# whxhcj/multimodal-S2UT

Measured on AMD Instinct MI355X. Metric: audio-frames/sec/node, mm_s2ut_transformer fp16, max-tokens 40000, 1/2/4/8 GPUs, higher is better.
Workload: dtype fp16; 1 GPU; mm_s2ut_transformer base (ViT-768 image feats, multimodal_attention+gate); model=mm_s2ut_transformer, parallelism=dp1, front_end=GPU fbank+CMVN in step

## Files before the change

### include/mms2ut.h

```cpp
#ifndef MMS2UT_H
#define MMS2UT_H

#include <hip/hip_runtime.h>
#include <stdint.h>

#ifdef __cplusplus
extern "C" {
#endif

typedef _Float16 mms2ut_half;

const char* mms2ut_last_error(void);
int mms2ut_stream_create(int priority, hipStream_t* out);
int mms2ut_stream_destroy(hipStream_t stream);
int mms2ut_version(void);

enum {
  MMS_EPI_F16 = 0,
  MMS_EPI_RELU_DROP = 1,
  MMS_EPI_DROP_RESID = 2,
  MMS_EPI_F32 = 3,
  MMS_EPI_GATE = 4,
  MMS_EPI_RELU_DROP_BWD = 5,
  MMS_EPI_F16_ACC = 6,
// ... 29 lines not shown
} mms2ut_gemm_args;

int mms2ut_gemm_f16(const mms2ut_gemm_args* args, hipStream_t stream);
int mms2ut_gemm_set_tall(int mode);

int mms2ut_gemm_set_skinny(int mode);
int mms2ut_gemm_skinny_debug(int scatter, int* xcc_out);
int mms2ut_gemm_set_epilogue(int staged);

typedef struct mms2ut_wgrad {
  const mms2ut_half* dy;
  int64_t lddy;
  const mms2ut_half* x;
  int64_t ldx;
  mms2ut_half* dW;
  mms2ut_half* db;
  int N, K;
} mms2ut_wgrad;
int mms2ut_wgrad_group(const mms2ut_wgrad* w, int n, int64_t rows, int max_blocks, hipStream_t stream);

int mms2ut_profile_begin(int max_launches);
int mms2ut_profile_end(float* total_ms, int* launches, double* flops);
int mms2ut_profile_bytes(double* bytes);
int mms2ut_profile_launches(float* ms, double* flops, int* cls, int n);
int mms2ut_profile_shapes(int* mnk, int n);
int mms2ut_profile_stamps(unsigned long long* stamps, long cap_blocks);
int mms2ut_profile_blocks(long* first_last, int n);
int mms2ut_wallclock_khz(int* khz);

int mms2ut_splitk_reduce(const float* slabs, int nsplit, int64_t slab, int rows, int cols,
                         void* out, int64_t ldo, int mode, float alpha, hipStream_t stream);
int mms2ut_splitk_reduce_bias(const float* slabs, int nsplit, int64_t slab, int rows, int cols,
                              mms2ut_half* out, int64_t ldo, const float* rs_slabs,
                              mms2ut_half* rs_out, hipStream_t stream);

typedef struct mms2ut_transpose_desc {
  int64_t src, dst;
  int32_t rows, cols, tile0, pad;
} mms2ut_transpose_desc;
int mms2ut_transpose_batch(const mms2ut_half* src, mms2ut_half* dst, const mms2ut_transpose_desc* descs,
                           int n, int total_tiles, hipStream_t stream);

int mms2ut_stream_wait(hipStream_t waiter, hipStream_t signaler);
int mms2ut_event_create(hipEvent_t* out);
int mms2ut_event_record(hipEvent_t event, hipStream_t stream);
int mms2ut_event_wait(hipStream_t stream, hipEvent_t event);
int mms2ut_event_destroy(hipEvent_t event);
int mms2ut_bind_step_seed(const uint64_t* delta);
int mms2ut_step_seed_advance(uint64_t* delta, uint64_t inc, hipStream_t stream);

int mms2ut_layernorm_fwd(const mms2ut_half* x, const mms2ut_half* gamma, const mms2ut_half* beta,
                         mms2ut_half* y, float* mean, float* rstd, int64_t rows, int D, float eps,
                         hipStream_t stream);
int mms2ut_layernorm_bwd(const mms2ut_half* dy, const mms2ut_half* x, const mms2ut_half* gamma,
                         const float* mean, const float* rstd, const mms2ut_half* dres,
                         mms2ut_half* dx, float* part, int64_t rows, int D, mms2ut_half* dxd,
                         float p, uint64_t seed, uint64_t offset, hipStream_t stream);
int mms2ut_layernorm_bwd_parts(int64_t rows);
int mms2ut_layernorm_bwd_nparts(int64_t rows, int D);
int mms2ut_layernorm_fwd_ex(const mms2ut_half* x, const mms2ut_half* gamma, const mms2ut_half* beta,
                            mms2ut_half* y, float* mean, float* rstd, int64_t rows, int D, float eps,
                            int64_t grp, int64_t grp_out, float p, uint64_t seed, uint64_t offset,
                            hipStream_t stream);
int mms2ut_layernorm_bwd_ex(const mms2ut_half* dy, const mms2ut_half* x, const mms2ut_half* gamma,
                            const float* mean, const float* rstd, const mms2ut_half* dres,
                            mms2ut_half* dx, float* part, int64_t rows, int D, mms2ut_half* dxd,
                            float p, uint64_t seed, uint64_t offset, int64_t dy_grp, int64_t dy_grp_out,
                            float dy_p, uint64_t dy_seed, uint64_t dy_offset, hipStream_t stream);
int mms2ut_colsum_parts(const float* part, int nparts, int ncol, mms2ut_half* out, int accumulate,
                        hipStream_t stream);
int mms2ut_colsum_f16(const mms2ut_half* x, int64_t rows, int cols, int64_t ld, float* part,
                      int nparts, hipStream_t stream);
int mms2ut_colsum_nparts(int64_t rows);

int mms2ut_attn_softmax_fwd(const mms2ut_half* S, mms2ut_half* P, mms2ut_half* Pd, int Z, int H,
                            int Tq, int Tk, int64_t ldS, const int32_t* key_len,
                            const uint8_t* key_mask, int64_t ld_mask, int causal,
                            int extra_key, float p, uint64_t seed, uint64_t offset,
                            hipStream_t stream);
int mms2ut_attn_softmax_bwd(const mms2ut_half* P, const mms2ut_half* dPd, mms2ut_half* dS, int Z,
                            int H, int Tq, int Tk, int64_t ldS, const int32_t* key_len, int causal,
                            int extra_key, float p, uint64_t seed, uint64_t offset,
                            hipStream_t stream);

typedef struct mms2ut_attn_args {
  const mms2ut_half* q;
  const mms2ut_half* k;
  const mms2ut_half* v;
  mms2ut_half* o;
  int64_t ldq, ldk, ldv, ldo;
  int64_t sqb, skb, svb, sob;
  int B, H, Tq, Tk, hd;
  const int32_t* key_len;
  int causal;
  float scale;
  float p;
  uint64_t seed, offset;
  float* lse;
} mms2ut_attn_args;

int mms2ut_mha_varlen_fwd(const mms2ut_attn_args* args, hipStream_t stream);
int mms2ut_mha_varlen_bwd(const mms2ut_attn_args* args, const mms2ut_half* dout, int64_t lddo,
                          int64_t sdob, float* Dd, mms2ut_half* dq, int64_t lddq, int64_t sdqb,
                          mms2ut_half* dk, int64_t lddk, int64_t sdkb, mms2ut_half* dv,
                          int64_t lddv, int64_t sdvb, hipStream_t stream);

int mms2ut_dropout_fwd(const mms2ut_half* x, mms2ut_half* y, int64_t n, float p, uint64_t seed,
                       uint64_t offset, hipStream_t stream);
int mms2ut_dropout_mask(uint8_t* keep, int64_t n, float p, uint64_t seed, uint64_t offset,
                        hipStream_t stream);
int mms2ut_encoder_embed_fwd(const mms2ut_half* h, const mms2ut_half* pos_table, const int32_t* len,
                             mms2ut_half* x, int B, int T, int D, float scale, float p,
                             uint64_t seed, uint64_t offset, hipStream_t stream);
int mms2ut_scale_dropout_bwd(const mms2ut_half* dx, mms2ut_half* dh, int64_t n, float scale,
                             float p, uint64_t seed, uint64_t offset, hipStream_t stream);
int mms2ut_token_embed_fwd(const int64_t* tok, const mms2ut_half* E, const mms2ut_half* pos_table,
                           mms2ut_half* x, int B, int T, int D, int pad_idx, float scale, float p,
                           uint64_t seed, uint64_t offset, hipStream_t stream);
int mms2ut_token_embed_bwd(const int64_t* tok, const mms2ut_half* dx, float* dE32, int B, int T,
                           int D, int V, int pad_idx, float scale, float p, uint64_t seed,
                           uint64_t offset, hipStream_t stream);
int mms2ut_add_f32_to_f16(const mms2ut_half* a, const float* b, mms2ut_half* out, int64_t n,
                          hipStream_t stream);
int mms2ut_glu_fwd(const mms2ut_half* x, mms2ut_half* y, int64_t rows, int C, hipStream_t stream);
int mms2ut_glu_bwd(const mms2ut_half* x, const mms2ut_half* dy, mms2ut_half* dx, int64_t rows,
                   int C, hipStream_t stream);
int mms2ut_im2col(const mms2ut_half* x, mms2ut_half* col, int B, int Tin, int Tout, int C, int k,
                  int stride, int pad, hipStream_t stream);
int mms2ut_im2col_ld(const mms2ut_half* x, mms2ut_half* col, int B, int Tin, int Tout, int C, int k,
                     int stride, int pad, int ldcol, hipStream_t stream);
int mms2ut_col2im(const mms2ut_half* dcol, mms2ut_half* dx, int B, int Tin, int Tout, int C, int k,
                  int stride, int pad, hipStream_t stream);
int mms2ut_gate_bwd(const mms2ut_half* dres, const mms2ut_half* merge, const mms2ut_half* g,
                    mms2ut_half* dpre, mms2ut_half* dmerge, int64_t rows, int D,
                    hipStream_t stream);
int mms2ut_copy2d(const mms2ut_half* src, int64_t lds, mms2ut_half* dst, int64_t ldd, int64_t rows,
                  int cols, hipStream_t stream);
int mms2ut_copy2d_pad(const mms2ut_half* src, int64_t lds, mms2ut_half* dst, int64_t ldd, int64_t rows,
                      int cols, int zcols, hipStream_t stream);
int mms2ut_add_f16(const mms2ut_half* a, const mms2ut_half* b, mms2ut_half* out, int64_t n,
                   hipStream_t stream);

#define MMS_LS_XENT_PARTS 512
int mms2ut_ls_xent_fwd(const mms2ut_half* logits, int64_t ld, const int64_t* target, int64_t rows,
                       int V, float eps, int pad_idx, float* lse, float* part, float* loss_out,
                       hipStream_t stream);
int mms2ut_ls_xent_fwd_log(const mms2ut_half* logits, int64_t ld, const int64_t* target, int64_t rows,
                           int V, float eps, int pad_idx, float* lse, float* part, float* acc, float* call_out,
                           hipStream_t stream);
int mms2ut_ls_xent_bwd(const mms2ut_half* logits, int64_t ld, const int64_t* target, int64_t rows,
                       int V, float eps, int pad_idx, const float* lse, const float* grad,
                       mms2ut_half* dlogits, hipStream_t stream);

enum {
  MMS_OST_MULT = 0, MMS_OST_GNORM = 1, MMS_OST_OVERFLOW = 2, MMS_OST_STEP = 3,
  MMS_OST_STEP_SIZE = 4, MMS_OST_LOSS_SCALE = 5, MMS_OST_ITER = 6, MMS_OST_LAST_OVERFLOW = 7,
  MMS_OST_LAST_RESCALE = 8, MMS_OST_CLIP_COEF = 9, MMS_OST_FATAL = 10, MMS_OST_LR = 11,
  MMS_OST_INCONSISTENT = 12, MMS_OST_SIZE = 16
};
int mms2ut_grad_sqnorm(const mms2ut_half* grad, int64_t n, float* part, int nparts,
                       hipStream_t stream);
int mms2ut_grad_norm_finalize(const float* part, int nparts, float* ost, const float* sample_size,
                              hipStream_t stream);
int mms2ut_optim_prepare(float* ost, float lr, float warmup_init_lr, float warmup_updates, float beta1,
                         float beta2, float clip_norm, float scale_window, float min_loss_scale,
                         hipStream_t stream);
// ... 46 lines not shown
int mms2ut_specaugment_f16(mms2ut_half* x, const int32_t* frame_off, int B, int Tmax, int nbins,
                           const int32_t* masks, int n_freq, int n_time, int use_const,
                           float mask_value, hipStream_t stream);
#define MMS_NOISE_SPLIT    8
#define MMS_NOISE_MAX_MIX  4
#define MMS_NOISE_WS_DOUBLES(B) ((int64_t)3 * (B) * MMS_NOISE_SPLIT)
int mms2ut_noise_mix_f32(float* wave, const int64_t* wave_off, int B,
                         const int16_t* bank, const int64_t* bank_off, int n_clips,
                         const int32_t* params, int n_mix, double* ws, hipStream_t stream);

enum { MMS_LAYER_ENC = 0, MMS_LAYER_DEC = 1 };
enum {
  MMS_SLOT_M1 = 0, MMS_SLOT_R1, MMS_SLOT_H1, MMS_SLOT_QKV, MMS_SLOT_LSE_SA, MMS_SLOT_O, MMS_SLOT_XA,
  MMS_SLOT_M2, MMS_SLOT_R2, MMS_SLOT_H2, MMS_SLOT_Q, MMS_SLOT_LSE_CA, MMS_SLOT_CO, MMS_SLOT_XB,
  MMS_SLOT_M3, MMS_SLOT_R3, MMS_SLOT_H3, MMS_SLOT_F1, MMS_SLOT_OUT, MMS_LAYER_NSLOT
};

typedef struct mms2ut_layer {
  int kind;
  int B, T, Tk, d, H, F;
  float eps;
  const int32_t* self_len;
  const int32_t* cross_len;
  const mms2ut_half *ln1_g, *ln1_b, *w_qkv, *b_qkv, *w_o, *b_o;
  const mms2ut_half *ln2_g, *ln2_b, *w_cq, *b_cq, *w_co, *b_co;
  const mms2ut_half* kv;
  int64_t ld_kv;
  const mms2ut_half *ln3_g, *ln3_b, *w_fc1, *b_fc1, *w_fc2, *b_fc2;
  const mms2ut_half *wt_qkv, *wt_o, *wt_cq, *wt_co, *wt_fc1, *wt_fc2;
  mms2ut_half *g_ln1, *g_w_qkv, *g_b_qkv, *g_w_o, *g_b_o;
  mms2ut_half *g_ln2, *g_w_cq, *g_b_cq, *g_w_co, *g_b_co;
  mms2ut_half *g_ln3, *g_w_fc1, *g_b_fc1, *g_w_fc2, *g_b_fc2;
  float p_drop, p_attn, p_act;
  uint64_t seed;
  uint64_t off_sa_attn, off_sa_res, off_ca_attn, off_ca_res, off_act, off_ffn_res;
  const mms2ut_half* x;
  void* saved;
} mms2ut_layer;

typedef struct mms2ut_layer_grad {
  const mms2ut_half* dy;
  const mms2ut_half* dy_drop;
  float emit_p;
  uint64_t emit_seed, emit_offset;
  mms2ut_half* dkv;
  int64_t ld_dkv;
  void* scratch;
  float* main_ws;
  int64_t main_ws_floats;
  float* side_ws;
  int64_t side_ws_floats;
  int side_blocks;
} mms2ut_layer_grad;

int mms2ut_layer_arena(const mms2ut_layer* layer, int64_t* offsets, int64_t* bytes);
int mms2ut_layer_scratch(const mms2ut_layer* layer, float emit_p, int64_t* dx_offsets, int64_t* bytes);
int mms2ut_layer_ws(const mms2ut_layer* layer, int64_t* main_floats, int64_t* side_floats);
int mms2ut_layer_fwd(const mms2ut_layer* layer, float* main_ws, int64_t main_ws_floats, hipStream_t stream);
int mms2ut_layer_bwd(const mms2ut_layer* layer, const mms2ut_layer_grad* grad, hipStream_t main,
                     hipStream_t side);
int mms2ut_wgrad_flush(hipStream_t main);

#define MMS_CONV_MAX 4
typedef struct mms2ut_conv1d_glu {
  int B, T, C, nlayers;
  int k[MMS_CONV_MAX];
  int cout[MMS_CONV_MAX];
  const mms2ut_half* w[MMS_CONV_MAX];
  const mms2ut_half* b[MMS_CONV_MAX];
  const mms2ut_half* wt[MMS_CONV_MAX];
  mms2ut_half* g_w[MMS_CONV_MAX];
  mms2ut_half* g_b[MMS_CONV_MAX];
  const mms2ut_half* x;
  void* saved;
} mms2ut_conv1d_glu;
int mms2ut_conv1d_glu_arena(const mms2ut_conv1d_glu* c, int64_t* out_offset, int64_t* bytes);
int mms2ut_conv1d_glu_scratch(const mms2ut_conv1d_glu* c, int64_t* dx_offset, int64_t* bytes);
int mms2ut_conv1d_glu_ws(const mms2ut_conv1d_glu* c, int64_t* main_floats, int64_t* side_floats);
int mms2ut_conv1d_glu_fwd(const mms2ut_conv1d_glu* c, float* main_ws, int64_t main_ws_floats, hipStream_t stream);
int mms2ut_conv1d_glu_bwd(const mms2ut_conv1d_glu* c, const mms2ut_half* dy, void* scratch, float* main_ws,
                          int64_t main_ws_floats, float* side_ws, int64_t side_ws_floats, int side_blocks,
                          hipStream_t main, hipStream_t side);

typedef struct mms2ut_gated_fusion {
  int B, Te, Ti, Di, d;
  int extra;
  int gate;
  int image_pre_norm;
  float eps;
  float p_img, p_txt, p_attn;
  uint64_t seed, off_img, off_txt, off_attn;
  const uint8_t* key_mask;
  int64_t ld_mask;
  const mms2ut_half *ln_g, *ln_b, *wq, *bq, *wkv, *bkv, *bias_kv, *wo, *bo, *wg, *bg;
  mms2ut_half *g_ln, *g_wq, *g_bq, *g_wkv, *g_bkv, *g_bias_kv, *g_wo, *g_bo, *g_wg, *g_bg;
  const mms2ut_half *wt_q, *wt_kv, *wt_o, *wt_g;
  const mms2ut_half* text;
  const mms2ut_half* img;
  void* saved;
} mms2ut_gated_fusion;
int mms2ut_gated_fusion_arena(const mms2ut_gated_fusion* f, int64_t* out_offset, int64_t* bytes);
int mms2ut_gated_fusion_scratch(const mms2ut_gated_fusion* f, int want_dimg, int64_t* offsets, int64_t* bytes);
int mms2ut_gated_fusion_ws(const mms2ut_gated_fusion* f, int64_t* main_floats, int64_t* side_floats);
int mms2ut_gated_fusion_fwd(const mms2ut_gated_fusion* f, float* main_ws, int64_t main_ws_floats, hipStream_t stream);
int mms2ut_gated_fusion_bwd(const mms2ut_gated_fusion* f, const mms2ut_half* dres, int want_dimg, void* scratch,
                            float* main_ws, int64_t main_ws_floats, float* side_ws, int64_t side_ws_floats,
                            int side_blocks, hipStream_t main, hipStream_t side);

enum { MMS_OP_LAYER = 0, MMS_OP_CONV1D_GLU = 1, MMS_OP_GATED_FUSION = 2 };
int mms2ut_workspace_size(int op, const void* desc, int64_t* sizes);

#ifdef __cplusplus
}
#endif
#endif
```

### multimodal-s2ut_amd/_lib.py

```python
import ctypes as C
import os
import struct

HERE = os.path.dirname(os.path.abspath(__file__))
LIB_PATH = os.environ.get("MMS2UT_LIB") or os.path.join(HERE, "lib", "libmms2ut_hip.so")

vp, i32, i64, u64, f32 = C.c_void_p, C.c_int, C.c_int64, C.c_uint64, C.c_float

EPI_F16, EPI_RELU_DROP, EPI_DROP_RESID, EPI_F32, EPI_GATE, EPI_RELU_DROP_BWD, EPI_F16_ACC, EPI_GELU_DROP, \
    EPI_GELU_DROP_BWD = range(9)


class GemmArgs(C.Structure):
    _fields_ = [
        ("A", vp), ("B", vp), ("C", vp),
        ("M", i32), ("N", i32), ("K", i32),
        ("a_kcontig", i32), ("b_kcontig", i32),
        ("lda", i64), ("ldb", i64), ("ldc", i64),
        ("batch", i32), ("bdiv", i32),
        ("sA1", i64), ("sA2", i64), ("sB1", i64), ("sB2", i64), ("sC1", i64), ("sC2", i64),
        ("splitk", i32),
        ("sCsplit", i64),
        ("epi", i32),
        ("alpha", f32),
# ... 58 lines not shown


CONV_MAX = 4


class ConvArgs(C.Structure):
    _fields_ = [("B", i32), ("T", i32), ("C", i32), ("nlayers", i32), ("k", i32 * CONV_MAX), ("cout", i32 * CONV_MAX)] + \
        [(n, vp * CONV_MAX) for n in ("w", "b", "wt", "g_w", "g_b")] + [("x", vp), ("saved", vp)]


class FusionArgs(C.Structure):
    _fields_ = [(n, i32) for n in ("B", "Te", "Ti", "Di", "d", "extra", "gate", "image_pre_norm")] + \
        [(n, f32) for n in ("eps", "p_img", "p_txt", "p_attn")] + [(n, u64) for n in ("seed", "off_img", "off_txt", "off_attn")] + \
        [("key_mask", vp), ("ld_mask", i64)] + \
        [(n, vp) for n in ("ln_g", "ln_b", "wq", "bq", "wkv", "bkv", "bias_kv", "wo", "bo", "wg", "bg",
                           "g_ln", "g_wq", "g_bq", "g_wkv", "g_bkv", "g_bias_kv", "g_wo", "g_bo", "g_wg", "g_bg",
                           "wt_q", "wt_kv", "wt_o", "wt_g", "text", "img", "saved")]


OP_LAYER, OP_CONV1D_GLU, OP_GATED_FUSION = range(3)


class WgradArgs(C.Structure):
    _fields_ = [("dy", vp), ("lddy", i64), ("x", vp), ("ldx", i64), ("dW", vp), ("db", vp), ("N", i32), ("K", i32)]


class LayerGradArgs(C.Structure):
    _fields_ = [("dy", vp), ("dy_drop", vp), ("emit_p", f32), ("emit_seed", u64), ("emit_offset", u64),
                ("dkv", vp), ("ld_dkv", i64), ("scratch", vp), ("main_ws", vp), ("main_ws_floats", i64),
                ("side_ws", vp), ("side_ws_floats", i64), ("side_blocks", i32)]


LAYER_GRAD_ARGS = _packer(LayerGradArgs)


SIGNATURES = {
    "mms2ut_last_error": (C.c_char_p, []),
    "mms2ut_version": (i32, []),
    "mms2ut_stream_create": (i32, [i32, vp]),
    "mms2ut_stream_destroy": (i32, [vp]),
    "mms2ut_event_create": (i32, [vp]),
    "mms2ut_event_record": (i32, [vp, vp]),
    "mms2ut_event_wait": (i32, [vp, vp]),
    "mms2ut_event_destroy": (i32, [vp]),
    "mms2ut_gemm_f16": (i32, [vp, vp]),
    "mms2ut_gemm_set_tall": (i32, [i32]),
    "mms2ut_gemm_set_skinny": (i32, [i32]),
    "mms2ut_gemm_skinny_debug": (i32, [i32, vp]),
    "mms2ut_gemm_set_epilogue": (i32, [i32]),
    "mms2ut_wgrad_group": (i32, [vp, i32, i64, i32, vp]),
    "mms2ut_wgrad_flush": (i32, [vp]),
    "mms2ut_profile_begin": (i32, [i32]),
    "mms2ut_profile_end": (i32, [C.POINTER(C.c_float), C.POINTER(C.c_int), C.POINTER(C.c_double)]),
    "mms2ut_profile_bytes": (i32, [C.POINTER(C.c_double)]),
    "mms2ut_profile_launches": (i32, [C.c_void_p, C.c_void_p, C.c_void_p, i32]),
    "mms2ut_profile_shapes": (i32, [C.c_void_p, i32]),
    "mms2ut_profile_stamps": (i32, [vp, C.c_long]),
    "mms2ut_profile_blocks": (i32, [C.c_void_p, i32]),
    "mms2ut_wallclock_khz": (i32, [C.POINTER(C.c_int)]),
    "mms2ut_grad_norm_check": (i32, [vp, i32, i32, vp, i32, vp]),
    "mms2ut_ctc_workspace_floats": (i32, [i32, i32, i32, C.POINTER(C.c_int64)]),
    "mms2ut_ctc_loss_fwd": (i32, [vp, i64, i32, i32, i32, vp, i64, i32, vp, vp, i32, i32, vp, vp, vp]),
    "mms2ut_ctc_loss_bwd": (i32, [vp, i64, i32, i32, i32, vp, i64, i32, vp, vp, i32, vp, vp, vp, i64, vp]),
    "mms2ut_scale_f16": (i32, [vp, i64, f32, vp]),
    "mms2ut_accum_f16_f32": (i32, [vp, vp, i64, vp]),
    "mms2ut_set_f32": (i32, [vp, i32, vp, vp]),
    "mms2ut_splitk_reduce": (i32, [vp, i32, i64, i32, i32, vp, i64, i32, f32, vp]),
    "mms2ut_splitk_reduce_bias": (i32, [vp, i32, i64, i32, i32, vp, i64, vp, vp, vp]),
    "mms2ut_transpose_batch": (i32, [vp, vp, vp, i32, i32, vp]),
    "mms2ut_layernorm_fwd": (i32, [vp, vp, vp, vp, vp, vp, i64, i32, f32, vp]),
    "mms2ut_layernorm_bwd": (i32, [vp, vp, vp, vp, vp, vp, vp, vp, i64, i32, vp, f32, u64, u64, vp]),
    "mms2ut_layernorm_bwd_parts": (i32, [i64]),
    "mms2ut_layernorm_bwd_nparts": (i32, [i64, i32]),
    "mms2ut_layernorm_fwd_ex": (i32, [vp, vp, vp, vp, vp, vp, i64, i32, f32, i64, i64, f32, u64, u64, vp]),
    "mms2ut_layernorm_bwd_ex": (i32, [vp, vp, vp, vp, vp, vp, vp, vp, i64, i32, vp, f32, u64, u64, i64, i64,
                                      f32, u64, u64, vp]),
    "mms2ut_colsum_parts": (i32, [vp, i32, i32, vp, i32, vp]),
    "mms2ut_colsum_f16": (i32, [vp, i64, i32, i64, vp, i32, vp]),
    "mms2ut_colsum_nparts": (i32, [i64]),
    "mms2ut_attn_softmax_fwd": (i32, [vp, vp, vp, i32, i32, i32, i32, i64, vp, vp, i64, i32, i32,
                                      f32, u64, u64, vp]),
    "mms2ut_attn_softmax_bwd": (i32, [vp, vp, vp, i32, i32, i32, i32, i64, vp, i32, i32, f32, u64,
                                      u64, vp]),
    "mms2ut_mha_varlen_fwd": (i32, [vp, vp]),
    "mms2ut_mha_varlen_bwd": (i32, [vp, vp, i64, i64, vp, vp, i64, i64, vp, i64, i64,
                                    vp, i64, i64, vp]),
    "mms2ut_dropout_fwd": (i32, [vp, vp, i64, f32, u64, u64, vp]),
    "mms2ut_dropout_mask": (i32, [vp, i64, f32, u64, u64, vp]),
    "mms2ut_encoder_embed_fwd": (i32, [vp, vp, vp, vp, i32, i32, i32, f32, f32, u64, u64, vp]),
    "mms2ut_scale_dropout_bwd": (i32, [vp, vp, i64, f32, f32, u64, u64, vp]),
    "mms2ut_token_embed_fwd": (i32, [vp, vp, vp, vp, i32, i32, i32, i32, f32, f32, u64, u64, vp]),
    "mms2ut_token_embed_bwd": (i32, [vp, vp, vp, i32, i32, i32, i32, i32, f32, f32, u64, u64, vp]),
    "mms2ut_add_f32_to_f16": (i32, [vp, vp, vp, i64, vp]),
    "mms2ut_add_f16": (i32, [vp, vp, vp, i64, vp]),
    "mms2ut_glu_fwd": (i32, [vp, vp, i64, i32, vp]),
    "mms2ut_glu_bwd": (i32, [vp, vp, vp, i64, i32, vp]),
    "mms2ut_im2col": (i32, [vp, vp, i32, i32, i32, i32, i32, i32, i32, vp]),
    "mms2ut_im2col_ld": (i32, [vp, vp, i32, i32, i32, i32, i32, i32, i32, i32, vp]),
    "mms2ut_col2im": (i32, [vp, vp, i32, i32, i32, i32, i32, i32, i32, vp]),
    "mms2ut_gate_bwd": (i32, [vp, vp, vp, vp, vp, i64, i32, vp]),
    "mms2ut_copy2d_pad": (i32, [vp, i64, vp, i64, i64, i32, i32, vp]),
    "mms2ut_copy2d": (i32, [vp, i64, vp, i64, i64, i32, vp]),
    "mms2ut_ls_xent_fwd": (i32, [vp, i64, vp, i64, i32, f32, i32, vp, vp, vp, vp]),
    "mms2ut_ls_xent_fwd_log": (i32, [vp, i64, vp, i64, i32, f32, i32, vp, vp, vp, vp, vp]),
    "mms2ut_ls_xent_bwd": (i32, [vp, i64, vp, i64, i32, f32, i32, vp, vp, vp, vp]),
    "mms2ut_grad_sqnorm": (i32, [vp, i64, vp, i32, vp]),
    "mms2ut_grad_norm_finalize": (i32, [vp, i32, vp, vp, vp]),
    "mms2ut_stream_wait": (i32, [vp, vp]),
    "mms2ut_bind_step_seed": (i32, [vp]),
    "mms2ut_step_seed_advance": (i32, [vp, u64, vp]),
    "mms2ut_optim_prepare": (i32, [vp, f32, f32, f32, f32, f32, f32, f32, f32, vp]),
    "mms2ut_adam_fp16_master": (i32, [vp, vp, vp, vp, vp, i64, vp, f32, f32, f32, f32, vp]),
    "mms2ut_fbank_frames": (i32, [vp, i32, vp, vp]),
    "mms2ut_fbank_f32": (i32, [vp, vp, vp, i32, i32, vp, vp, i32, vp, vp]),
    "mms2ut_fbank_cmvn_collate": (i32, [vp, vp, i32, i32, i32, i32, vp, vp, vp]),
    "mms2ut_specaugment_f16": (i32, [vp, vp, i32, i32, i32, vp, i32, i32, i32, f32, vp]),
    "mms2ut_noise_mix_f32": (i32, [vp, vp, i32, vp, vp, i32, vp, i32, vp, vp]),
    "mms2ut_layer_arena": (i32, [vp, vp, vp]),
    "mms2ut_layer_scratch": (i32, [vp, f32, vp, vp]),
    "mms2ut_layer_ws": (i32, [vp, vp, vp]),
    "mms2ut_layer_fwd": (i32, [vp, vp, i64, vp]),
    "mms2ut_layer_bwd": (i32, [vp, vp, vp, vp]),
    "mms2ut_gated_fusion_arena": (i32, [vp, vp, vp]),
    "mms2ut_gated_fusion_scratch": (i32, [vp, i32, vp, vp]),
    "mms2ut_gated_fusion_ws": (i32, [vp, vp, vp]),
    "mms2ut_gated_fusion_fwd": (i32, [vp, vp, i64, vp]),
    "mms2ut_gated_fusion_bwd": (i32, [vp, vp, i32, vp, vp, i64, vp, i64, i32, vp, vp]),
    "mms2ut_workspace_size": (i32, [i32, vp, vp]),
    "mms2ut_conv1d_glu_arena": (i32, [vp, vp, vp]),
    "mms2ut_conv1d_glu_scratch": (i32, [vp, vp, vp]),
    "mms2ut_conv1d_glu_ws": (i32, [vp, vp, vp]),
    "mms2ut_conv1d_glu_fwd": (i32, [vp, vp, i64, vp]),
    "mms2ut_conv1d_glu_bwd": (i32, [vp, vp, vp, vp, i64, vp, i64, i32, vp, vp]),
    "mms2ut_log_softmax_step": (i32, [vp, i64, i64, i32, i32, i32, i32, vp, vp]),
    "mms2ut_kv_cache_gather": (i32, [vp, vp, vp, i32, i32, i32, i32, i32, i32, vp]),
    "mms2ut_decode_self_attn": (i32, [vp, i64, vp, vp, i32, i32, i32, i32, vp, vp, i64, i64, vp, i64, f32, vp]),
    "mms2ut_decode_embed": (i32, [vp, vp, vp, vp, i32, vp, i32, i32, f32, vp]),
    "mms2ut_splitk_epilogue_f16": (i32, [vp, i32, i64, i32, i32, vp, vp, i64, i32, vp, i64, vp]),
    "mms2ut_beam_topk": (i32, [vp, vp, i64, i32, i32, i32, i32, i32, vp, vp, vp, vp, vp]),
    "mms2ut_splitk_epilogue_ln_f16": (i32, [vp, i32, i64, i32, i32, vp, vp, i64, vp, i64, vp, vp, f32, vp, i64,
                                            vp]),
}

_lib = None


class HipError(RuntimeError):
    pass


def load():
    global _lib
    if _lib is not None:
        return _lib
    if not os.path.exists(LIB_PATH):
        raise HipError(f"libmms2ut_hip.so not found at {LIB_PATH}; run "
                       f"`python multimodal-s2ut_amd/build.py` (hipcc, gfx950)")
    lib = C.CDLL(LIB_PATH)
    for name, (res, args) in SIGNATURES.items():
        fn = getattr(lib, name)
        fn.restype = res
        fn.argtypes = args
    _lib = lib
    return lib


def call(name, *args):
    rc = getattr(_lib or load(), name)(*args)
    if rc != 0:
        raise HipError(f"{name} failed ({rc}): {_lib.mms2ut_last_error().decode()}")
    return rc
```

### multimodal-s2ut_amd/csrc/layers.hip

```cpp
#include <math.h>
#include <stdlib.h>

#include <algorithm>

#include "common.h"
#include "../../include/mms2ut.h"

namespace {

constexpr int64_t kAlign = 256;

int64_t al(int64_t b) { return (b + kAlign - 1) / kAlign * kAlign; }

struct Dims {
  bool dec;
  int64_t R, Rk, d, F, BHT, BHTk;
};

Dims dims_of(const mms2ut_layer* L) {
  Dims D;
  D.dec = L->kind == MMS_LAYER_DEC;
  D.R = (int64_t)L->B * L->T;
  D.Rk = (int64_t)L->B * L->Tk;
  D.d = L->d;
// ... 560 lines not shown
    const int k = c->k[i], N = c->cout[i];
    mms2ut_half* col = at<mms2ut_half>(A, off, i * CA_N + CA_COL);
    mms2ut_half* y = at<mms2ut_half>(A, off, i * CA_N + CA_Y);
    mms2ut_half* g = at<mms2ut_half>(A, off, i * CA_N + CA_G);
    if ((rc = mms2ut_im2col_ld(x, col, c->B, (int)D.Tin[i], (int)D.Tout[i], (int)D.C[i], k, 2, k / 2, (int)D.kp[i], s)))
      return rc;
    const mms2ut_half* W = c->w[i];
    if (D.kp[i] != D.ck[i]) {
      mms2ut_half* Wp = at<mms2ut_half>(A, off, i * CA_N + CA_WP);
      if ((rc = mms2ut_copy2d_pad(W, D.ck[i], Wp, D.kp[i], N, (int)D.ck[i], (int)(D.kp[i] - D.ck[i]), s))) return rc;
      W = Wp;
    }
    if ((rc = linear(cx, col, W, c->b[i], y, D.rows[i], N, D.kp[i]))) return rc;
    if ((rc = mms2ut_glu_fwd(y, g, D.rows[i], N / 2, s))) return rc;
    x = g;
  }
  return 0;
}

extern "C" int mms2ut_conv1d_glu_bwd(const mms2ut_conv1d_glu* c, const mms2ut_half* dy, void* scratch,
                                     float* main_ws, int64_t main_ws_floats, float* side_ws,
                                     int64_t side_ws_floats, int side_blocks, hipStream_t main, hipStream_t side) {
  if (int rc = conv_check(c)) return rc;
  MMS_REQUIRE(dy && scratch && c->saved, "conv1d_glu_bwd: null gradient / scratch / arena");
  if (!side) side = main;
  const ConvDims D = conv_dims(c);
  int64_t sz[MMS_CONV_MAX * CA_N], off[MMS_CONV_MAX * CA_N];
  conv_arena_sizes(c, D, sz);
  layout(sz, MMS_CONV_MAX * CA_N, off);
  int64_t ssz[MMS_CONV_MAX * CS_N + 1], so[MMS_CONV_MAX * CS_N + 1];
  conv_scratch_sizes(c, D, ssz);
  layout(ssz, MMS_CONV_MAX * CS_N + 1, so);
  void* A = c->saved;
  void* S = scratch;
  const Ctx cx{main, side, main_ws, main_ws_floats, side_ws, side_ws_floats, at<float>(S, so, MMS_CONV_MAX * CS_N),
               nullptr, nullptr, false};
  const mms2ut_half* dg = dy;
  int rc;
  for (int i = D.n - 1; i >= 0; --i) {
    const int k = c->k[i], N = c->cout[i];
    const mms2ut_half* col = at<mms2ut_half>(A, off, i * CA_N + CA_COL);
    mms2ut_half* dyi = at<mms2ut_half>(S, so, i * CS_N + CS_DY);
    if ((rc = mms2ut_glu_bwd(at<mms2ut_half>(A, off, i * CA_N + CA_Y), dg, dyi, D.rows[i], N / 2, main))) return rc;
    if (c->g_w[i]) {
      if (conv_group_ok(c, D, i)) {
        if ((rc = fork(cx))) return rc;
        mms2ut_wgrad w{dyi, N, col, D.kp[i], c->g_w[i], c->g_b[i], N, (int)D.ck[i]};
        if ((rc = mms2ut_wgrad_group(&w, 1, D.rows[i], side == main ? 0 : side_blocks, side))) return rc;
      } else if ((rc = wgrad(cx, dyi, N, col, D.kp[i], c->g_w[i], c->g_b[i], D.rows[i], N, D.ck[i]))) {
        return rc;
      }
    }
    if (i == 0) break;
    mms2ut_half* dcol = at<mms2ut_half>(S, so, i * CS_N + CS_DCOL);
    mms2ut_half* dx = at<mms2ut_half>(S, so, i * CS_N + CS_DX);
    if ((rc = dgrad(cx, dyi, N, c->w[i], c->wt[i], dcol, D.rows[i], N, D.ck[i]))) return rc;
    if ((rc = mms2ut_col2im(dcol, dx, c->B, (int)D.Tin[i], (int)D.Tout[i], (int)D.C[i], k, 2, k / 2, main))) return rc;
    dg = dx;
  }
  return 0;
}

namespace {

bool wgrad_group_ok(const mms2ut_half* dy, int64_t lddy, const mms2ut_half* x, int64_t ldx, const mms2ut_half* dW,
                    int64_t M, int64_t N, int64_t K) {
  auto al16 = [](const void* p) { return ((uintptr_t)p & 15) == 0; };
  return ((N + 127) / 128) * ((K + 127) / 128) >= 256 && N % 8 == 0 && K % 8 == 0 && lddy % 8 == 0 && ldx % 8 == 0 &&
         al16(dy) && al16(x) && al16(dW) && M * std::max(lddy, ldx) * 2 < (1LL << 31);
}

int wgrad_auto(const Ctx& c, const mms2ut_half* dy, int64_t lddy, const mms2ut_half* x, int64_t ldx, mms2ut_half* dW,
               mms2ut_half* db, int64_t M, int64_t N, int64_t K, int side_blocks) {
  if (wgrad_group_ok(dy, lddy, x, ldx, dW, M, N, K)) {
    int rc = fork(c);
    if (rc) return rc;
    mms2ut_wgrad w{dy, lddy, x, ldx, dW, db, (int)N, (int)K};
    return mms2ut_wgrad_group(&w, 1, M, c.side == c.main ? 0 : side_blocks, c.side);
  }
  return wgrad(c, dy, lddy, x, ldx, dW, db, M, N, K);
}

struct FusDims {
  int64_t B, Te, Ti, Tk, Di, d, Rt, Ri, Rk, ldS;
  bool extra, gate, pre, ln_fused;
};

FusDims fus_dims(const mms2ut_gated_fusion* f) {
  FusDims D;
  D.B = f->B; D.Te = f->Te; D.Ti = f->Ti; D.Di = f->Di; D.d = f->d;
  D.extra = f->extra != 0; D.gate = f->gate != 0; D.pre = f->image_pre_norm != 0;
  D.Tk = D.Ti + (D.extra ? 1 : 0);
  D.Rt = D.B * D.Te; D.Ri = D.B * D.Ti; D.Rk = D.B * D.Tk;
  D.ldS = (D.Tk + 7) / 8 * 8;
  D.ln_fused = D.pre && D.Di % 256 == 0 && D.Di <= 1024;
  return D;
}

enum { FA_IM = 0, FA_IR, FA_IMGN, FA_IMGD, FA_TEXTD, FA_Q, FA_KV, FA_S, FA_P, FA_PD, FA_O, FA_MERGE, FA_G, FA_OUT, FA_N };
void fus_arena_sizes(const mms2ut_gated_fusion* f, const FusDims& D, int64_t* sz) {
  for (int i = 0; i < FA_N; ++i) sz[i] = 0;
  const int64_t h = 2;
  if (D.pre) sz[FA_IM] = sz[FA_IR] = D.Ri * 4;
  if (!D.ln_fused && (D.pre || f->p_img > 0.f)) sz[FA_IMGN] = D.Ri * D.Di * h;
  if (D.ln_fused || D.extra) sz[FA_IMGD] = D.Rk * D.Di * h;
  if (f->p_txt > 0.f) sz[FA_TEXTD] = D.Rt * D.d * h;
  sz[FA_Q] = D.Rt * D.d * h;
  sz[FA_KV] = D.Rk * 2 * D.d * h;
  sz[FA_S] = sz[FA_P] = D.Rt * D.ldS * h;
  if (f->p_attn > 0.f) sz[FA_PD] = sz[FA_P];
  sz[FA_O] = D.Rt * D.d * h;
  if (D.gate) { sz[FA_MERGE] = D.Rt * 2 * D.d * h; sz[FA_G] = D.Rt * D.d * h; }
  sz[FA_OUT] = D.Rt * D.d * h;
}

enum { FS_DPRE = 0, FS_DMERGE, FS_DO, FS_DQ, FS_DKV, FS_DPD, FS_DIMGD, FS_DIMG, FS_DIMGIN, FS_DTEXT, FS_LNP, FS_KVP,
       FS_BPART, FS_N };
void fus_scratch_sizes(const mms2ut_gated_fusion* f, const FusDims& D, int want_dimg, int64_t* sz) {
  for (int i = 0; i < FS_N; ++i) sz[i] = 0;
  const int64_t h = 2;
  if (D.gate) { sz[FS_DPRE] = D.Rt * D.d * h; sz[FS_DMERGE] = D.Rt * 2 * D.d * h; }
  sz[FS_DO] = sz[FS_DQ] = D.Rt * D.d * h;
  sz[FS_DKV] = D.Rk * 2 * D.d * h;
  sz[FS_DPD] = D.Rt * D.ldS * h;
  if (D.pre || want_dimg) {
    sz[FS_DIMGD] = D.Rk * D.Di * h;
    sz[FS_DIMG] = D.Ri * D.Di * h;
    sz[FS_DIMGIN] = D.Ri * D.Di * h;
    if (D.pre) sz[FS_LNP] = (int64_t)mms2ut_layernorm_bwd_nparts(D.Ri, (int)D.Di) * 2 * D.Di * 4;
  }
  sz[FS_DTEXT] = D.Rt * D.d * h;
  if (D.extra) sz[FS_KVP] = (int64_t)mms2ut_colsum_nparts(D.B) * 2 * D.d * 4;
  sz[FS_BPART] = (int64_t)mms2ut_colsum_nparts(std::max(D.Rt, D.Rk)) * 2 * D.d * 4;
}

int fus_check(const mms2ut_gated_fusion* f) {
  MMS_REQUIRE(f && f->B >= 1 && f->Te >= 1 && f->Ti >= 1, "gated_fusion: B, Te, Ti must be >= 1");
  MMS_REQUIRE(f->d % 8 == 0 && f->Di % 8 == 0 && f->d > 0 && f->Di > 0, "gated_fusion: d=%d Di=%d (multiples of 8)", f->d, f->Di);
  MMS_REQUIRE(f->wq && f->bq && f->wkv && f->bkv && f->wo && f->bo, "gated_fusion: projection weights / biases required");
  MMS_REQUIRE(!f->extra || f->bias_kv, "gated_fusion: multimodal attention needs bias_kv");
  MMS_REQUIRE(!f->gate || (f->wg && f->bg), "gated_fusion: the gate needs its weight and bias");
  MMS_REQUIRE(!f->image_pre_norm || (f->ln_g && f->ln_b), "gated_fusion: image_pre_norm needs the LayerNorm");
  return 0;
}

mms2ut_gemm_args batched(const mms2ut_half* A, const mms2ut_half* B_, void* C, int M, int N, int K, int a_kc, int b_kc,
                         int64_t lda, int64_t ldb, int64_t ldc, int batch, int64_t sA, int64_t sB, int64_t sC,
                         float alpha) {
  mms2ut_gemm_args a = gemm_args();
  a.A = A; a.B = B_; a.C = C;
  a.M = M; a.N = N; a.K = K;
  a.a_kcontig = a_kc; a.b_kcontig = b_kc;
  a.lda = lda; a.ldb = ldb; a.ldc = ldc;
  a.batch = batch; a.bdiv = 1;
  a.sA1 = sA; a.sB1 = sB; a.sC1 = sC;
  a.sA2 = a.sB2 = a.sC2 = 0;
  a.alpha = alpha;
  return a;
}

int zero_rows(mms2ut_half* p, int64_t pitch_elems, int64_t width_elems, int64_t rows, hipStream_t s) {
  return mms2ut_copy2d_pad(nullptr, 0, p, pitch_elems, rows, 0, (int)width_elems, s);
}

}

extern "C" int mms2ut_gated_fusion_arena(const mms2ut_gated_fusion* f, int64_t* out_offset, int64_t* bytes) {
  if (int rc = fus_check(f)) return rc;
  MMS_REQUIRE(bytes, "gated_fusion_arena: null");
  const FusDims D = fus_dims(f);
  int64_t sz[FA_N], off[FA_N];
  fus_arena_sizes(f, D, sz);
  *bytes = layout(sz, FA_N, off);
  if (out_offset) *out_offset = off[FA_OUT];
  return 0;
}

extern "C" int mms2ut_gated_fusion_scratch(const mms2ut_gated_fusion* f, int want_dimg, int64_t* offsets, int64_t* bytes) {
  if (int rc = fus_check(f)) return rc;
  MMS_REQUIRE(bytes, "gated_fusion_scratch: null");
  const FusDims D = fus_dims(f);
  int64_t sz[FS_N], off[FS_N];
  fus_scratch_sizes(f, D, want_dimg, sz);
  *bytes = layout(sz, FS_N, off);
  if (offsets) {
    offsets[0] = off[FS_DTEXT];
    offsets[1] = want_dimg ? (D.pre ? off[FS_DIMGIN] : (D.extra ? off[FS_DIMG] : off[FS_DIMGD])) : -1;
  }
  return 0;
}

extern "C" int mms2ut_gated_fusion_ws(const mms2ut_gated_fusion* f, int64_t* main_floats, int64_t* side_floats) {
  if (int rc = fus_check(f)) return rc;
  MMS_REQUIRE(main_floats && side_floats, "gated_fusion_ws: null");
  const FusDims D = fus_dims(f);
  int64_t mw = 0, sw = 0;
  auto fw = [&](int64_t M, int64_t N, int64_t K) {
    const int s = fixup_splits(M, N, K);
    if (s > 1) mw = std::max(mw, (int64_t)s * M * N);
  };
  auto ww = [&](int64_t M, int64_t N, int64_t K) {
    const int s = wgrad_splits(((N + 127) / 128) * ((K + 127) / 128), M);
    sw = std::max(sw, (int64_t)s * N * K + (int64_t)s * N);
  };
  const int64_t d = D.d;
  fw(D.Rt, d, d); fw(D.Rk, 2 * d, D.Di); fw(D.Rt, d, d); fw(D.Rt, d, 2 * d);
  fw(D.Rt, 2 * d, d); fw(D.Rt, d, d); fw(D.Rk, D.Di, 2 * d); fw(D.Rt, d, d);
  ww(D.Rt, d, 2 * d); ww(D.Rt, d, d); ww(D.Rk, 2 * d, D.Di); ww(D.Rt, d, d);
  *main_floats = mw;
  *side_floats = sw;
  return 0;
}

extern "C" int mms2ut_gated_fusion_fwd(const mms2ut_gated_fusion* f, float* main_ws, int64_t main_ws_floats,
                                       hipStream_t s) {
  if (int rc = fus_check(f)) return rc;
  MMS_REQUIRE(f->text && f->img && f->saved, "gated_fusion_fwd: null text / image / arena");
  const FusDims D = fus_dims(f);
  int64_t sz[FA_N], off[FA_N];
  fus_arena_sizes(f, D, sz);
  layout(sz, FA_N, off);
  void* A = f->saved;
  auto H_ = [&](int slot) { return at<mms2ut_half>(A, off, slot); };
  const Ctx c{s, s, main_ws, main_ws_floats, nullptr, 0, nullptr};
  const int64_t d = D.d, Di = D.Di;
  int rc;
  const mms2ut_half* imgd;
  if (D.ln_fused) {
    if (D.extra && (rc = zero_rows(H_(FA_IMGD) + D.Ti * Di, D.Tk * Di, Di, D.B, s))) return rc;
    if ((rc = mms2ut_layernorm_fwd_ex(f->img, f->ln_g, f->ln_b, H_(FA_IMGD), at<float>(A, off, FA_IM),
                                      at<float>(A, off, FA_IR), D.Ri, (int)Di, f->eps, D.extra ? D.Ti : 0,
                                      D.extra ? D.Tk : 0, f->p_img, f->seed, f->off_img, s))) return rc;
    imgd = H_(FA_IMGD);
  } else {
    const mms2ut_half* imgn = f->img;
    if (D.pre) {
      if ((rc = mms2ut_layernorm_fwd(f->img, f->ln_g, f->ln_b, H_(FA_IMGN), at<float>(A, off, FA_IM),
                                     at<float>(A, off, FA_IR), D.Ri, (int)Di, f->eps, s))) return rc;
      imgn = H_(FA_IMGN);
    }
    if (f->p_img > 0.f) {
      if ((rc = mms2ut_dropout_fwd(imgn, H_(FA_IMGN), D.Ri * Di, f->p_img, f->seed, f->off_img, s))) return rc;
      imgn = H_(FA_IMGN);
    }
    if (D.extra) {
      if ((rc = mms2ut_copy2d_pad(imgn, D.Ti * Di, H_(FA_IMGD), D.Tk * Di, D.B, (int)(D.Ti * Di),
                                  (int)((D.Tk - D.Ti) * Di), s)))
        return rc;
      imgd = H_(FA_IMGD);
    } else {
      imgd = imgn;
    }
  }
  const mms2ut_half* textd = f->text;
  if (f->p_txt > 0.f) {
    if ((rc = mms2ut_dropout_fwd(f->text, H_(FA_TEXTD), D.Rt * d, f->p_txt, f->seed, f->off_txt, s))) return rc;
    textd = H_(FA_TEXTD);
  }
  mms2ut_half *q = H_(FA_Q), *kv = H_(FA_KV), *O = H_(FA_O);
  if ((rc = linear(c, textd, f->wq, f->bq, q, D.Rt, d, d))) return rc;
  if ((rc = linear(c, imgd, f->wkv, f->bkv, kv, D.Rk, 2 * d, Di))) return rc;
  if (D.extra && (rc = mms2ut_copy2d(f->bias_kv, 0, kv + D.Ti * 2 * d, D.Tk * 2 * d, D.B, (int)(2 * d), s))) return rc;
  const float scale = (float)pow((double)d, -0.5);
  mms2ut_half *S = H_(FA_S), *P = H_(FA_P), *Pd = f->p_attn > 0.f ? H_(FA_PD) : P;
  {
    mms2ut_gemm_args a = batched(q, kv, S, (int)D.Te, (int)D.Tk, (int)d, 1, 1, d, 2 * d, D.ldS, (int)D.B, D.Te * d,
                                 D.Tk * 2 * d, D.Te * D.ldS, scale);
    if ((rc = mms2ut_gemm_f16(&a, s))) return rc;
  }
  if ((rc = mms2ut_attn_softmax_fwd(S, P, Pd, (int)D.B, 1, (int)D.Te, (int)D.Tk, D.ldS, nullptr, f->key_mask,
                                    f->key_mask ? f->ld_mask : 0, 0, D.extra ? 1 : 0, f->p_attn,
                                    f->p_attn > 0.f ? f->seed : 0, f->p_attn > 0.f ? f->off_attn : 0, s))) return rc;
  {
    mms2ut_gemm_args a = batched(Pd, kv + d, O, (int)D.Te, (int)d, (int)D.Tk, 1, 0, D.ldS, 2 * d, d, (int)D.B,
                                 D.Te * D.ldS, D.Tk * 2 * d, D.Te * d, 1.f);
    if ((rc = mms2ut_gemm_f16(&a, s))) return rc;
  }
  mms2ut_half* out = H_(FA_OUT);
  if (D.gate) {
    mms2ut_half* merge = H_(FA_MERGE);
    if ((rc = gemm_nt(c, O, d, f->wo, d, 1, merge, 2 * d, D.Rt, d, d, MMS_EPI_F16, f->bo, nullptr, 0, 0.f, 0, 0, d)))
      return rc;
    if ((rc = mms2ut_copy2d(textd, d, merge + d, 2 * d, D.Rt, (int)d, s))) return rc;
    mms2ut_gemm_args a = gemm_args();
    a.A = merge; a.B = f->wg; a.C = out;
    a.M = (int)D.Rt; a.N = (int)d; a.K = (int)(2 * d);
    a.a_kcontig = 1; a.b_kcontig = 1;
    a.lda = 2 * d; a.ldb = 2 * d; a.ldc = d;
    a.epi = MMS_EPI_GATE; a.bias = f->bg; a.aux = merge; a.ldaux = 2 * d; a.out2 = H_(FA_G); a.ldo2 = d;
    a.ld_rng = d;
    const int sp = fixup_splits(D.Rt, d, 2 * d);
    if (sp > 1) {
      MMS_REQUIRE(main_ws && main_ws_floats >= (int64_t)sp * D.Rt * d, "gated_fusion_fwd: main workspace too small");
      a.splitk = sp; a.splitk_ws = main_ws; a.splitk_ws_floats = main_ws_floats;
    }
    return mms2ut_gemm_f16(&a, s);
  }
  return linear(c, O, f->wo, f->bo, out, D.Rt, d, d, MMS_EPI_DROP_RESID, textd);
}

extern "C" int mms2ut_gated_fusion_bwd(const mms2ut_gated_fusion* f, const mms2ut_half* dres, int want_dimg,
                                       void* scratch, float* main_ws, int64_t main_ws_floats, float* side_ws,
                                       int64_t side_ws_floats, int side_blocks, hipStream_t main, hipStream_t side) {
  if (int rc = fus_check(f)) return rc;
  MMS_REQUIRE(dres && scratch && f->saved, "gated_fusion_bwd: null gradient / scratch / arena");
  if (!side) side = main;
  const FusDims D = fus_dims(f);
  int64_t sz[FA_N], off[FA_N], ssz[FS_N], so[FS_N];
  fus_arena_sizes(f, D, sz);
  layout(sz, FA_N, off);
  fus_scratch_sizes(f, D, want_dimg, ssz);
  layout(ssz, FS_N, so);
  void* A = f->saved;
  void* S = scratch;
  auto H_ = [&](int slot) { return at<mms2ut_half>(A, off, slot); };
  auto SH = [&](int slot) { return at<mms2ut_half>(S, so, slot); };
  auto SF = [&](int slot) { return at<float>(S, so, slot); };
  const Ctx c{main, side, main_ws, main_ws_floats, side_ws, side_ws_floats, SF(FS_BPART), nullptr, nullptr, false};
  const int64_t d = D.d, Di = D.Di;
  const mms2ut_half* textd = f->p_txt > 0.f ? H_(FA_TEXTD) : f->text;
  const mms2ut_half* imgd = (D.ln_fused || D.extra) ? H_(FA_IMGD) : (!D.ln_fused && (D.pre || f->p_img > 0.f) ? H_(FA_IMGN) : f->img);
  int rc;
  const mms2ut_half *dOp = dres, *dtext = dres;
  int64_t lddop = d, lddtext = d;
  if (D.gate) {
    mms2ut_half *dpre = SH(FS_DPRE), *dmerge = SH(FS_DMERGE);
    if ((rc = mms2ut_gate_bwd(dres, H_(FA_MERGE), H_(FA_G), dpre, dmerge, D.Rt, (int)d, main))) return rc;
    if ((rc = wgrad_auto(c, dpre, d, H_(FA_MERGE), 2 * d, f->g_wg, f->g_bg, D.Rt, d, 2 * d, side_blocks))) return rc;
    if ((rc = dgrad(c, dpre, d, f->wg, f->wt_g, dmerge, D.Rt, d, 2 * d, MMS_EPI_F16_ACC))) return rc;
    dOp = dmerge; lddop = 2 * d;
    dtext = dmerge + d; lddtext = 2 * d;
  }
  if ((rc = wgrad_auto(c, dOp, lddop, H_(FA_O), d, f->g_wo, f->g_bo, D.Rt, d, d, side_blocks))) return rc;
  mms2ut_half* dO = SH(FS_DO);
  if ((rc = dgrad(c, dOp, lddop, f->wo, f->wt_o, dO, D.Rt, d, d))) return rc;
  const float scale = (float)pow((double)d, -0.5);
  const mms2ut_half *q = H_(FA_Q), *kv = H_(FA_KV), *P = H_(FA_P), *Pd = f->p_attn > 0.f ? H_(FA_PD) : P;
  mms2ut_half *dq = SH(FS_DQ), *dkv = SH(FS_DKV), *dPd = SH(FS_DPD);
  const int B = (int)D.B, Te = (int)D.Te, Tk = (int)D.Tk;
  const int64_t sS = D.Te * D.ldS;
  {
    mms2ut_gemm_args a = batched(dO, kv + d, dPd, Te, Tk, (int)d, 1, 1, d, 2 * d, D.ldS, B, D.Te * d, D.Tk * 2 * d, sS, 1.f);
    if ((rc = mms2ut_gemm_f16(&a, main))) return rc;
    a = batched(Pd, dO, dkv + d, Tk, (int)d, Te, 0, 0, D.ldS, d, 2 * d, B, sS, D.Te * d, D.Tk * 2 * d, 1.f);
    if ((rc = mms2ut_gemm_f16(&a, main))) return rc;
  }
  if ((rc = mms2ut_attn_softmax_bwd(P, dPd, dPd, B, 1, Te, Tk, D.ldS, nullptr, 0, 0, f->p_attn,
                                    f->p_attn > 0.f ? f->seed : 0, f->p_attn > 0.f ? f->off_attn : 0, main))) return rc;
  {
    mms2ut_gemm_args a = batched(dPd, kv, dq, Te, (int)d, Tk, 1, 0, D.ldS, 2 * d, d, B, sS, D.Tk * 2 * d, D.Te * d, scale);
    if ((rc = mms2ut_gemm_f16(&a, main))) return rc;
    a = batched(dPd, q, dkv, Tk, (int)d, Te, 0, 0, D.ldS, d, 2 * d, B, sS, D.Te * d, D.Tk * 2 * d, scale);
    if ((rc = mms2ut_gemm_f16(&a, main))) return rc;
  }
  if (D.extra) {
    mms2ut_half* rows = dkv + D.Ti * 2 * d;
    const int np = mms2ut_colsum_nparts(D.B);
    if ((rc = mms2ut_colsum_f16(rows, D.B, (int)(2 * d), D.Tk * 2 * d, SF(FS_KVP), np, main))) return rc;
    if ((rc = mms2ut_colsum_parts(SF(FS_KVP), np, (int)(2 * d), f->g_bias_kv, 0, main))) return rc;
    if ((rc = zero_rows(rows, D.Tk * 2 * d, 2 * d, D.B, main))) return rc;
  }
  if ((rc = wgrad_auto(c, dkv, 2 * d, imgd, Di, f->g_wkv, f->g_bkv, D.Rk, 2 * d, Di, side_blocks))) return rc;
  if (D.ln_fused) {
    mms2ut_half* dimgd = SH(FS_DIMGD);
    if ((rc = dgrad(c, dkv, 2 * d, f->wkv, f->wt_kv, dimgd, D.Rk, 2 * d, Di))) return rc;
    if ((rc = mms2ut_layernorm_bwd_ex(dimgd, f->img, f->ln_g, at<float>(A, off, FA_IM), at<float>(A, off, FA_IR), nullptr,
                                      want_dimg ? SH(FS_DIMGIN) : nullptr, SF(FS_LNP), D.Ri, (int)Di, nullptr, 0.f, 0, 0,
                                      D.extra ? D.Ti : 0, D.extra ? D.Tk : 0, f->p_img, f->p_img > 0.f ? f->seed : 0,
                                      f->p_img > 0.f ? f->off_img : 0, main))) return rc;
    if ((rc = fork(c)) ||
        (rc = mms2ut_colsum_parts(SF(FS_LNP), mms2ut_layernorm_bwd_nparts(D.Ri, (int)Di), (int)(2 * Di), f->g_ln, 0, side)))
      return rc;
  } else if (D.pre || want_dimg) {
    mms2ut_half* dimgd = SH(FS_DIMGD);
    if ((rc = dgrad(c, dkv, 2 * d, f->wkv, f->wt_kv, dimgd, D.Rk, 2 * d, Di))) return rc;
    mms2ut_half* dimg = dimgd;
    if (D.extra) {
      dimg = SH(FS_DIMG);
      if ((rc = mms2ut_copy2d(dimgd, D.Tk * Di, dimg, D.Ti * Di, D.B, (int)(D.Ti * Di), main))) return rc;
    }
    if (f->p_img > 0.f && (rc = mms2ut_dropout_fwd(dimg, dimg, D.Ri * Di, f->p_img, f->seed, f->off_img, main))) return rc;
    if (D.pre) {
      if ((rc = ln_bwd(c, dimg, f->img, f->ln_g, at<float>(A, off, FA_IM), at<float>(A, off, FA_IR), nullptr,
                       want_dimg ? SH(FS_DIMGIN) : nullptr, nullptr, 0.f, 0, 0, SF(FS_LNP), f->g_ln, D.Ri, (int)Di)))
        return rc;
    }
  }
  if ((rc = wgrad_auto(c, dq, d, textd, d, f->g_wq, f->g_bq, D.Rt, d, d, side_blocks))) return rc;
  mms2ut_half* dtt = SH(FS_DTEXT);
  if ((rc = mms2ut_copy2d(dtext, lddtext, dtt, d, D.Rt, (int)d, main))) return rc;
  if ((rc = dgrad(c, dq, d, f->wq, f->wt_q, dtt, D.Rt, d, d, MMS_EPI_F16_ACC))) return rc;
  if (f->p_txt > 0.f && (rc = mms2ut_dropout_fwd(dtt, dtt, D.Rt * d, f->p_txt, f->seed, f->off_txt, main))) return rc;
  return 0;
}

extern "C" int mms2ut_workspace_size(int op, const void* desc, int64_t* sizes) {
  MMS_REQUIRE(desc && sizes, "workspace_size: null");
  int rc;
  switch (op) {
    case MMS_OP_LAYER: {
      const mms2ut_layer* L = static_cast<const mms2ut_layer*>(desc);
      if ((rc = mms2ut_layer_arena(L, nullptr, &sizes[0])) || (rc = mms2ut_layer_scratch(L, 0.f, nullptr, &sizes[1])))
        return rc;
      return mms2ut_layer_ws(L, &sizes[2], &sizes[3]);
    }
    case MMS_OP_CONV1D_GLU: {
      const mms2ut_conv1d_glu* c = static_cast<const mms2ut_conv1d_glu*>(desc);
      if ((rc = mms2ut_conv1d_glu_arena(c, nullptr, &sizes[0])) || (rc = mms2ut_conv1d_glu_scratch(c, nullptr, &sizes[1])))
        return rc;
      return mms2ut_conv1d_glu_ws(c, &sizes[2], &sizes[3]);
    }
    case MMS_OP_GATED_FUSION: {
      const mms2ut_gated_fusion* f = static_cast<const mms2ut_gated_fusion*>(desc);
      if ((rc = mms2ut_gated_fusion_arena(f, nullptr, &sizes[0])) ||
          (rc = mms2ut_gated_fusion_scratch(f, 0, nullptr, &sizes[1])))
        return rc;
      return mms2ut_gated_fusion_ws(f, &sizes[2], &sizes[3]);
    }
    default:
      mms::set_error("workspace_size: unknown op %d", op);
      return 1;
  }
}
```

### multimodal-s2ut_amd/csrc/ops.hip

```cpp
#include <stdlib.h>

#include "common.h"
#include "../../include/mms2ut.h"

namespace {

inline int grid_for(long n, int block, int cap = 8192) {
  long g = (n + block - 1) / block;
  if (g > cap) g = cap;
  if (g < 1) g = 1;
  return (int)g;
}

MMS_DEV h16x4 ld4(const h16* p) { return *reinterpret_cast<const h16x4*>(p); }
MMS_DEV void st4(h16* p, float a, float b, float c, float d) {
  *reinterpret_cast<h16x4*>(p) = h16x4{(h16)a, (h16)b, (h16)c, (h16)d};
}

template <int CPL>
__global__ void __launch_bounds__(256) ln_fwd_kernel(const h16* __restrict__ x, const h16* __restrict__ g,
                                                     const h16* __restrict__ b, h16* __restrict__ y,
                                                     float* __restrict__ mean_out, float* __restrict__ rstd_out,
                                                     long rows, int D, float eps, long grp, long grp_out,
                                                     float p, uint32_t thresh, uint64_t seed, uint64_t offset) {
// ... 326 lines not shown
          if (dxd) {
            bool kp[4] = {true, true, true, true};
            if (emit_hi) mms_keep4_hi(emit_mix, offset + (uint64_t)off, thresh, kp);
            else if (thresh) mms_keep4(seed, offset + (uint64_t)off, thresh, kp);
            st4(dxd + (long)off, kp[0] ? o[0] * dscale : 0.f, kp[1] ? o[1] * dscale : 0.f, kp[2] ? o[2] * dscale : 0.f,
                kp[3] ? o[3] * dscale : 0.f);
          }
        }
      }
    }
  }
#pragma unroll
  for (int c = 0; c < C; ++c)
    *reinterpret_cast<f32x4*>(&red[w][0][(lane + 64 * c) * 4]) = f32x4{dg[c][0], dg[c][1], dg[c][2], dg[c][3]};
#pragma unroll
  for (int c = 0; c < C; ++c)
    *reinterpret_cast<f32x4*>(&red[w][1][(lane + 64 * c) * 4]) = f32x4{db[c][0], db[c][1], db[c][2], db[c][3]};
  __syncthreads();
  float* out = part + (long)blockIdx.x * 2 * D;
  for (int i = threadIdx.x; i < 2 * D / 4; i += 256) {
    const int which = (4 * i) / D, j = 4 * i - which * D;
    f32x4 t = *reinterpret_cast<const f32x4*>(&red[0][which][j]);
#pragma unroll
    for (int v = 1; v < 4; ++v) t += *reinterpret_cast<const f32x4*>(&red[v][which][j]);
    *reinterpret_cast<f32x4*>(out + 4 * i) = t;
  }
}

__global__ void __launch_bounds__(1024) colsum_parts_kernel(const float* __restrict__ part, int nparts, int ncol,
                                                            h16* __restrict__ out, int accumulate) {
  __shared__ float red[64][17];
  const int lane = threadIdx.x & 63, w = threadIdx.x >> 6;
  const int col = lane & 15, slot = 4 * w + (lane >> 4);
  const int c = blockIdx.x * 16 + col;
  float s = 0.f;
  if (c < ncol) {
    for (int p0 = slot; p0 < nparts; p0 += 64 * 16) {
      float v[16];
#pragma unroll
      for (int i = 0; i < 16; ++i) {
        const int p = p0 + 64 * i;
        v[i] = p < nparts ? part[(long)p * ncol + c] : 0.f;
      }
#pragma unroll
      for (int i = 0; i < 16; ++i) s += v[i];
    }
  }
  red[slot][col] = s;
  __syncthreads();
  if (threadIdx.x < 16 && blockIdx.x * 16 + (int)threadIdx.x < ncol) {
    float t = 0.f;
#pragma unroll 8
    for (int i = 0; i < 64; ++i) t += red[i][threadIdx.x];
    const int cc = blockIdx.x * 16 + threadIdx.x;
    if (accumulate) t += (float)out[cc];
    out[cc] = (h16)t;
  }
}

constexpr int COLSUM_MAX_SPLITS = 64;
__global__ void __launch_bounds__(256) colsum_f16_kernel(const h16* __restrict__ x, long rows, int cols, long ld,
                                                         float* __restrict__ part, int splits) {
  __shared__ f32x4 red[4][64];
  const int lane = threadIdx.x & 63, w = threadIdx.x >> 6;
  const int c = (blockIdx.x * 64 + lane) * 4;
  const long per = (rows + splits - 1) / splits;
  const long r0 = (long)blockIdx.y * per, r1 = min(rows, r0 + per);
  f32x4 s = {0.f, 0.f, 0.f, 0.f};
  if (c < cols) {
#pragma unroll 4
    for (long r = r0 + w; r < r1; r += 4) {
      h16x4 v = ld4(x + r * ld + c);
      s += f32x4{(float)v[0], (float)v[1], (float)v[2], (float)v[3]};
    }
  }
  red[w][lane] = s;
  __syncthreads();
  if (w == 0 && c < cols) {
    const f32x4 t = red[0][lane] + red[1][lane] + red[2][lane] + red[3][lane];
    *reinterpret_cast<f32x4*>(part + (long)blockIdx.y * cols + c) = t;
  }
}

MMS_DEV bool key_valid(int j, int i, int Tk, int klen, const uint8_t* km, int causal, int extra_key) {
  if (j >= Tk) return false;
  if (extra_key && j == Tk - 1) return true;
  if (j >= klen) return false;
  if (km && km[j]) return false;
  if (causal && j > i) return false;
  return true;
}

template <int CPL>
__global__ void __launch_bounds__(256) softmax_fwd_kernel(const h16* __restrict__ S, h16* __restrict__ P,
                                                          h16* __restrict__ Pd, int Z, int H, int Tq, int Tk,
                                                          long ldS, const int* __restrict__ key_len,
                                                          const uint8_t* __restrict__ key_mask, long ld_mask,
                                                          int causal, int extra_key, float p, uint32_t thresh,
                                                          uint64_t seed, uint64_t offset) {
  if (thresh) seed = mms_step_seed(seed);
  const int lane = threadIdx.x & 63;
  const long row = (long)blockIdx.x * 4 + (threadIdx.x >> 6);
  if (row >= (long)Z * Tq) return;
  const int z = (int)(row / Tq), i = (int)(row % Tq);
  const int b = z / H;
  const int klen = key_len ? key_len[b] : Tk;
  const uint8_t* km = key_mask ? key_mask + (long)b * ld_mask : nullptr;
  const h16* sr = S + row * ldS;
  float v[CPL][4];
  float mx = -INFINITY;
#pragma unroll
  for (int c = 0; c < CPL; ++c) {
    const int j0 = (lane + c * 64) * 4;
    if (j0 < Tk) {
      h16x4 t = ld4(sr + j0);
#pragma unroll
      for (int e = 0; e < 4; ++e) {
        const int j = j0 + e;
        v[c][e] = key_valid(j, i, Tk, klen, km, causal, extra_key) ? (float)t[e] : -INFINITY;
        mx = fmaxf(mx, v[c][e]);
      }
    } else {
#pragma unroll
      for (int e = 0; e < 4; ++e) v[c][e] = -INFINITY;
    }
  }
  mx = wave_max(mx);
  float s = 0.f;
#pragma unroll
  for (int c = 0; c < CPL; ++c)
#pragma unroll
    for (int e = 0; e < 4; ++e) {
      const float ex = (v[c][e] == -INFINITY) ? 0.f : __expf(v[c][e] - mx);
      v[c][e] = ex;
      s += ex;
    }
  s = wave_sum(s);
  const float inv = s > 0.f ? 1.f / s : 0.f;
  const float ds = thresh ? 1.f / (1.f - p) : 1.f;
  h16* pr = P + row * ldS;
  h16* pdr = Pd + row * ldS;
#pragma unroll
  for (int c = 0; c < CPL; ++c) {
    const int j0 = (lane + c * 64) * 4;
    if (j0 < Tk) {
      float o[4], od[4];
#pragma unroll
      for (int e = 0; e < 4; ++e) {
        o[e] = (j0 + e < Tk) ? v[c][e] * inv : 0.f;
        od[e] = o[e];
        if (thresh) {
          const bool keep = mms_keep(seed, offset + (uint64_t)row * Tk + (j0 + e), thresh);
          od[e] = keep ? o[e] * ds : 0.f;
        }
      }
      st4(pr + j0, o[0], o[1], o[2], o[3]);
      if (thresh) st4(pdr + j0, od[0], od[1], od[2], od[3]);
    }
  }
}

template <int CPL>
__global__ void __launch_bounds__(256) softmax_bwd_kernel(const h16* __restrict__ P, const h16* __restrict__ dPd,
                                                          h16* __restrict__ dS, int Z, int H, int Tq, int Tk,
                                                          long ldS, float p, uint32_t thresh, uint64_t seed,
                                                          uint64_t offset) {
  if (thresh) seed = mms_step_seed(seed);
  const int lane = threadIdx.x & 63;
  const long row = (long)blockIdx.x * 4 + (threadIdx.x >> 6);
  if (row >= (long)Z * Tq) return;
  const float ds = thresh ? 1.f / (1.f - p) : 1.f;
  float pv[CPL][4], gv[CPL][4];
  float s = 0.f;
#pragma unroll
  for (int c = 0; c < CPL; ++c) {
    const int j0 = (lane + c * 64) * 4;
    if (j0 < Tk) {
      h16x4 a = ld4(P + row * ldS + j0), g = ld4(dPd + row * ldS + j0);
#pragma unroll
      for (int e = 0; e < 4; ++e) {
        const int j = j0 + e;
        float m = ds;
        if (thresh && j < Tk) m = mms_keep(seed, offset + (uint64_t)row * Tk + j, thresh) ? ds : 0.f;
        pv[c][e] = (j < Tk) ? (float)a[e] : 0.f;
        gv[c][e] = (j < Tk) ? (float)g[e] * m : 0.f;
        s += pv[c][e] * gv[c][e];
      }
    } else {
#pragma unroll
      for (int e = 0; e < 4; ++e) { pv[c][e] = 0.f; gv[c][e] = 0.f; }
    }
  }
  s = wave_sum(s);
#pragma unroll
  for (int c = 0; c < CPL; ++c) {
    const int j0 = (lane + c * 64) * 4;
    if (j0 < Tk) {
      float o[4];
#pragma unroll
      for (int e = 0; e < 4; ++e) o[e] = pv[c][e] * (gv[c][e] - s);
      st4(dS + row * ldS + j0, o[0], o[1], o[2], o[3]);
    }
  }
  (void)Z; (void)H;
}

__global__ void dropout_kernel(const h16* __restrict__ x, h16* __restrict__ y, long n, float p,
                               uint32_t thresh, uint64_t seed, uint64_t offset) {
  if (thresh) seed = mms_step_seed(seed);
  const float ds = 1.f / (1.f - p);
  const MmsSite site = mms_site(seed, offset, offset + (uint64_t)n - 1);
  for (long i = blockIdx.x * (long)blockDim.x + threadIdx.x; i < n; i += (long)gridDim.x * blockDim.x) {
    const float v = (float)x[i];
    y[i] = (h16)(mms_keep_site(site, seed, offset + i, thresh) ? v * ds : 0.f);
  }
}

__global__ void dropout_mask_kernel(uint8_t* keep, long n, uint32_t thresh, uint64_t seed, uint64_t offset) {
  if (thresh) seed = mms_step_seed(seed);
  for (long i = blockIdx.x * (long)blockDim.x + threadIdx.x; i < n; i += (long)gridDim.x * blockDim.x)
    keep[i] = thresh ? (uint8_t)mms_keep(seed, offset + i, thresh) : 1;
}

__global__ void encoder_embed_kernel(const h16* __restrict__ h, const h16* __restrict__ pos,
                                     const int* __restrict__ len, h16* __restrict__ x, int B, int T,
                                     int D, float scale, float p, uint32_t thresh, uint64_t seed,
                                     uint64_t offset) {
  if (thresh) seed = mms_step_seed(seed);
  const long n4 = (long)B * T * (D / 4);
  const float ds = thresh ? 1.f / (1.f - p) : 1.f;
  const MmsSite site = thresh ? mms_site(seed, offset, offset + (uint64_t)n4 * 4 - 1) : MmsSite{false, 0u};
  for (long i = blockIdx.x * (long)blockDim.x + threadIdx.x; i < n4; i += (long)gridDim.x * blockDim.x) {
    const long e0 = i * 4;
    const long bt = e0 / D;
    const int d0 = (int)(e0 % D);
    const int b = (int)(bt / T), t = (int)(bt % T);
    const int pidx = (t < len[b]) ? t + 2 : 1;
    h16x4 hv = ld4(h + e0), pv = ld4(pos + (long)pidx * D + d0);
    float o[4];
#pragma unroll
    for (int e = 0; e < 4; ++e) {
      float v = scale * (float)hv[e] + (float)pv[e];
      if (thresh) v = mms_keep_site(site, seed, offset + e0 + e, thresh) ? v * ds : 0.f;
      o[e] = v;
    }
    st4(x + e0, o[0], o[1], o[2], o[3]);
  }
}

__global__ void scale_dropout_bwd_kernel(const h16* __restrict__ dx, h16* __restrict__ dh, long n,
                                         float scale, float p, uint32_t thresh, uint64_t seed,
                                         uint64_t offset) {
  if (thresh) seed = mms_step_seed(seed);
  const float ds = thresh ? 1.f / (1.f - p) : 1.f;
  const MmsSite site = thresh ? mms_site(seed, offset, offset + (uint64_t)n - 1) : MmsSite{false, 0u};
  for (long i = blockIdx.x * (long)blockDim.x + threadIdx.x; i < n; i += (long)gridDim.x * blockDim.x) {
    float v = (float)dx[i] * scale;
    if (thresh) v = mms_keep_site(site, seed, offset + i, thresh) ? v * ds : 0.f;
    dh[i] = (h16)v;
  }
}

__global__ void token_embed_fwd_kernel(const int64_t* __restrict__ tok, const h16* __restrict__ E,
                                       const h16* __restrict__ pos, h16* __restrict__ x, int B, int T,
                                       int D, int pad, float scale, float p, uint32_t thresh,
                                       uint64_t seed, uint64_t offset) {
  if (thresh) seed = mms_step_seed(seed);
  const int lane = threadIdx.x & 63;
  const long bt = (long)blockIdx.x * 4 + (threadIdx.x >> 6);
  if (bt >= (long)B * T) return;
  const int b = (int)(bt / T), t = (int)(bt % T);
  const int64_t tk = tok[bt];
  int cnt = 0;
  for (int j = lane; j <= t; j += 64) cnt += (tok[(long)b * T + j] != pad);
  cnt = (int)wave_sum((float)cnt);
  const int pidx = (tk != pad) ? cnt + pad : pad;
  const float ds = thresh ? 1.f / (1.f - p) : 1.f;
  for (int d0 = lane * 4; d0 < D; d0 += 256) {
    h16x4 ev = ld4(E + tk * D + d0), pv = ld4(pos + (long)pidx * D + d0);
    float o[4];
#pragma unroll
    for (int e = 0; e < 4; ++e) {
      float v = scale * (float)ev[e] + (float)pv[e];
      if (thresh) v = mms_keep(seed, offset + bt * D + d0 + e, thresh) ? v * ds : 0.f;
      o[e] = v;
    }
    st4(x + bt * D + d0, o[0], o[1], o[2], o[3]);
// ... 310 lines not shown
  const long rpb = 8L * ln16_iters(rows);
  return (int)((rows + rpb - 1) / rpb);
}

extern "C" int mms2ut_layernorm_bwd(const h16* dy, const h16* x, const h16* gamma, const float* mean,
                                    const float* rstd, const h16* dres, h16* dx, float* part,
                                    int64_t rows, int D, h16* dxd, float p, uint64_t seed,
                                    uint64_t offset, hipStream_t s) {
  MMS_REQUIRE(!dxd || dx, "layernorm_bwd: dxd needs dx");
  MMS_REQUIRE(p < 1.f, "layernorm_bwd: p must be < 1");
  const uint32_t thresh = mms_drop_thresh(p);
  MMS_REQUIRE(D % 4 == 0 && D <= 1024, "layernorm_bwd: D must be a multiple of 4 and <= 1024");
  if (rows == 0) return 0;
  const int nb = mms2ut_layernorm_bwd_nparts(rows, D);
  if (ln16_path(D)) {
    MMS_REQUIRE(rows * D < (1LL << 31), "layernorm_bwd: rows * D must be < 2^31 (32-bit row offsets)");
#define CASE(C) case C: hipLaunchKernelGGL((ln_bwd_w_kernel<C>), dim3(nb), dim3(256), 0, s, dy, x, gamma, mean, \
                                           rstd, dres, dx, part, (long)rows, D, dxd, p, thresh, seed, offset, 0L, \
                                           0L, 0.f, 0u, (uint64_t)0, (uint64_t)0, ln16_iters(rows)); break;
    switch (D / 256) { CASE(1) CASE(2) CASE(3) CASE(4) }
#undef CASE
    return mms::check_launch("layernorm_bwd_w");
  }
  return pick_cpl(D / 4, [&](auto C) {
    constexpr int CPL = decltype(C)::value;
    if constexpr (CPL <= 4) {
      hipLaunchKernelGGL((ln_bwd_kernel<CPL>), dim3(nb), dim3(256), 0, s, dy, x, gamma, mean, rstd,
                         dres, dx, part, (long)rows, D, dxd, p, thresh, seed, offset);
      return mms::check_launch("layernorm_bwd");
    } else {
      mms::set_error("layernorm_bwd: D too large");
      return 1;
    }
  });
}

extern "C" int mms2ut_layernorm_bwd_ex(const h16* dy, const h16* x, const h16* gamma, const float* mean,
                                       const float* rstd, const h16* dres, h16* dx, float* part,
                                       int64_t rows, int D, h16* dxd, float p, uint64_t seed, uint64_t offset,
                                       int64_t dy_grp, int64_t dy_grp_out, float dy_p, uint64_t dy_seed,
                                       uint64_t dy_offset, hipStream_t s) {
  MMS_REQUIRE(!dxd || dx, "layernorm_bwd_ex: dxd needs dx");
  MMS_REQUIRE(p < 1.f && dy_p < 1.f, "layernorm_bwd_ex: p must be < 1");
  MMS_REQUIRE(D % 256 == 0 && D <= 1024, "layernorm_bwd_ex: D must be a multiple of 256 and <= 1024");
  MMS_REQUIRE(dy_grp >= 0 && (dy_grp == 0 || dy_grp_out >= dy_grp), "layernorm_bwd_ex: need dy_grp_out >= dy_grp");
  if (rows == 0) return 0;
  const int nb = mms2ut_layernorm_bwd_nparts(rows, D);
  const uint32_t thresh = mms_drop_thresh(p), thin = mms_drop_thresh(dy_p);
  MMS_REQUIRE(rows * D < (1LL << 31) && (dy_grp == 0 || (rows / dy_grp + 1) * dy_grp_out * D < (1LL << 31)),
              "layernorm_bwd_ex: row offsets must fit 32 bits");
#define CASE(C) case C: hipLaunchKernelGGL((ln_bwd_w_kernel<C>), dim3(nb), dim3(256), 0, s, dy, x, gamma, mean, \
                                           rstd, dres, dx, part, (long)rows, D, dxd, p, thresh, seed, offset, \
                                           (long)dy_grp, (long)dy_grp_out, dy_p, thin, dy_seed, dy_offset, \
                                           ln16_iters(rows)); break;
  switch (D / 256) { CASE(1) CASE(2) CASE(3) CASE(4) }
#undef CASE
  return mms::check_launch("layernorm_bwd_ex");
}

extern "C" int mms2ut_colsum_parts(const float* part, int nparts, int ncol, h16* out, int accumulate,
                                   hipStream_t s) {
  if (ncol == 0) return 0;
  hipLaunchKernelGGL(colsum_parts_kernel, dim3((ncol + 15) / 16), dim3(1024), 0, s, part, nparts,
                     ncol, out, accumulate);
  return mms::check_launch("colsum_parts");
}

extern "C" int mms2ut_colsum_nparts(int64_t rows) {
  long sp = (rows + 63) / 64;
  if (sp > COLSUM_MAX_SPLITS) sp = COLSUM_MAX_SPLITS;
  return sp < 1 ? 1 : (int)sp;
}

extern "C" int mms2ut_colsum_f16(const h16* x, int64_t rows, int cols, int64_t ld, float* part,
                                 int nparts, hipStream_t s) {
  MMS_REQUIRE(cols % 4 == 0 && ld % 4 == 0, "colsum_f16: cols/ld must be multiples of 4");
  MMS_REQUIRE(nparts == mms2ut_colsum_nparts(rows), "colsum_f16: nparts mismatch");
  if (rows == 0) return 0;
  dim3 grid((cols / 4 + 63) / 64, nparts);
  hipLaunchKernelGGL(colsum_f16_kernel, grid, dim3(256), 0, s, x, (long)rows, cols, (long)ld, part, nparts);
  return mms::check_launch("colsum_f16");
}

extern "C" int mms2ut_attn_softmax_fwd(const h16* S, h16* P, h16* Pd, int Z, int H, int Tq, int Tk,
                                       int64_t ldS, const int32_t* key_len, const uint8_t* key_mask,
                                       int64_t ld_mask, int causal, int extra_key,
                                       float p, uint64_t seed, uint64_t offset, hipStream_t s) {
  MMS_REQUIRE(ldS % 4 == 0 && ldS >= Tk, "softmax: ldS must be a multiple of 4 and >= Tk");
  MMS_REQUIRE(p < 1.f, "softmax: p must be < 1");
  const long rows = (long)Z * Tq;
  if (rows == 0) return 0;
  const uint32_t th = mms_drop_thresh(p);
  return pick_cpl((Tk + 3) / 4, [&](auto C) {
    hipLaunchKernelGGL((softmax_fwd_kernel<decltype(C)::value>), dim3((rows + 3) / 4), dim3(256), 0, s,
                       S, P, Pd, Z, H, Tq, Tk, (long)ldS, key_len, key_mask, (long)ld_mask, causal,
                       extra_key, p, th, seed, offset);
    return mms::check_launch("attn_softmax_fwd");
  });
}

extern "C" int mms2ut_attn_softmax_bwd(const h16* P, const h16* dPd, h16* dS, int Z, int H, int Tq,
                                       int Tk, int64_t ldS, const int32_t* key_len, int causal,
                                       int extra_key, float p, uint64_t seed, uint64_t offset,
                                       hipStream_t s) {
  MMS_REQUIRE(ldS % 4 == 0 && ldS >= Tk, "softmax_bwd: ldS must be a multiple of 4 and >= Tk");
  const long rows = (long)Z * Tq;
  if (rows == 0) return 0;
  const uint32_t th = mms_drop_thresh(p);
  (void)key_len; (void)causal; (void)extra_key;
  return pick_cpl((Tk + 3) / 4, [&](auto C) {
    hipLaunchKernelGGL((softmax_bwd_kernel<decltype(C)::value>), dim3((rows + 3) / 4), dim3(256), 0, s,
                       P, dPd, dS, Z, H, Tq, Tk, (long)ldS, p, th, seed, offset);
    return mms::check_launch("attn_softmax_bwd");
  });
}

extern "C" int mms2ut_dropout_fwd(const h16* x, h16* y, int64_t n, float p, uint64_t seed,
                                  uint64_t offset, hipStream_t s) {
  MMS_REQUIRE(p < 1.f, "dropout: p must be < 1");
  if (n == 0) return 0;
  const uint32_t th = mms_drop_thresh(p);
  if (!th) {
    if (x != y) return hipMemcpyAsync(y, x, n * 2, hipMemcpyDeviceToDevice, s) == hipSuccess ? 0 : 1;
    return 0;
  }
  hipLaunchKernelGGL(dropout_kernel, dim3(grid_for(n, 256)), dim3(256), 0, s, x, y, (long)n, p, th, seed, offset);
  return mms::check_launch("dropout_fwd");
}

extern "C" int mms2ut_dropout_mask(uint8_t* keep, int64_t n, float p, uint64_t seed, uint64_t offset,
                                   hipStream_t s) {
  if (n == 0) return 0;
  hipLaunchKernelGGL(dropout_mask_kernel, dim3(grid_for(n, 256)), dim3(256), 0, s, keep, (long)n,
                     mms_drop_thresh(p), seed, offset);
  return mms::check_launch("dropout_mask");
}

extern "C" int mms2ut_encoder_embed_fwd(const h16* h, const h16* pos, const int32_t* len, h16* x, int B,
                                        int T, int D, float scale, float p, uint64_t seed,
                                        uint64_t offset, hipStream_t s) {
  MMS_REQUIRE(D % 4 == 0, "encoder_embed: D must be a multiple of 4");
  const long n4 = (long)B * T * (D / 4);
  if (n4 == 0) return 0;
  hipLaunchKernelGGL(encoder_embed_kernel, dim3(grid_for(n4, 256)), dim3(256), 0, s, h, pos, len, x, B,
                     T, D, scale, p, mms_drop_thresh(p), seed, offset);
  return mms::check_launch("encoder_embed_fwd");
}

extern "C" int mms2ut_scale_dropout_bwd(const h16* dx, h16* dh, int64_t n, float scale, float p,
                                        uint64_t seed, uint64_t offset, hipStream_t s) {
  if (n == 0) return 0;
  hipLaunchKernelGGL(scale_dropout_bwd_kernel, dim3(grid_for(n, 256)), dim3(256), 0, s, dx, dh, (long)n,
                     scale, p, mms_drop_thresh(p), seed, offset);
  return mms::check_launch("scale_dropout_bwd");
}

extern "C" int mms2ut_token_embed_fwd(const int64_t* tok, const h16* E, const h16* pos, h16* x, int B,
                                      int T, int D, int pad_idx, float scale, float p, uint64_t seed,
                                      uint64_t offset, hipStream_t s) {
  MMS_REQUIRE(D % 4 == 0, "token_embed: D must be a multiple of 4");
  const long n = (long)B * T;
  if (n == 0) return 0;
  hipLaunchKernelGGL(token_embed_fwd_kernel, dim3((n + 3) / 4), dim3(256), 0, s, tok, E, pos, x, B, T,
                     D, pad_idx, scale, p, mms_drop_thresh(p), seed, offset);
  return mms::check_launch("token_embed_fwd");
}

extern "C" int mms2ut_token_embed_bwd(const int64_t* tok, const h16* dx, float* dE32, int B, int T,
                                      int D, int V, int pad_idx, float scale, float p, uint64_t seed,
                                      uint64_t offset, hipStream_t s) {
  MMS_REQUIRE(D > 0 && D <= 64 * 8 * TEB_PASS && D % 8 == 0 && V > 0,
              "token_embed_bwd: D=%d (max %d, a multiple of 8) V=%d", D, 64 * 8 * TEB_PASS, V);
  MMS_REQUIRE(((uintptr_t)dx & 15) == 0, "token_embed_bwd: dx must be 16-B aligned");
  const long n = (long)B * T;
  if (n == 0) return 0;
  hipLaunchKernelGGL(token_embed_bwd_kernel, dim3(V), dim3(TEB_NT), 0, s, tok, dx, dE32, n, D,
                     pad_idx, scale, p, mms_drop_thresh(p), seed, offset);
  return mms::check_launch("token_embed_bwd");
}

extern "C" int mms2ut_add_f32_to_f16(const h16* a, const float* b, h16* out, int64_t n, hipStream_t s) {
  if (n == 0) return 0;
  hipLaunchKernelGGL(add_f32_to_f16_kernel, dim3(grid_for(n, 256)), dim3(256), 0, s, a, b, out, (long)n);
  return mms::check_launch("add_f32_to_f16");
}

extern "C" int mms2ut_add_f16(const h16* a, const h16* b, h16* out, int64_t n, hipStream_t s) {
  if (n == 0) return 0;
  hipLaunchKernelGGL(add_f16_kernel, dim3(grid_for(n, 256)), dim3(256), 0, s, a, b, out, (long)n);
  return mms::check_launch("add_f16");
}

extern "C" int mms2ut_glu_fwd(const h16* x, h16* y, int64_t rows, int C, hipStream_t s) {
  MMS_REQUIRE(C % 4 == 0, "glu: C must be a multiple of 4");
  const long n4 = (long)rows * (C / 4);
  if (n4 == 0) return 0;
  hipLaunchKernelGGL(glu_fwd_kernel, dim3(grid_for(n4, 256)), dim3(256), 0, s, x, y, (long)rows, C);
// ... 81 lines not shown
```

### multimodal-s2ut_amd/kernels.py

```python
import atexit
import ctypes
import math
import os

import torch

from . import _lib
from ._lib import GemmArgs, call

EPI_F16, EPI_RELU_DROP, EPI_DROP_RESID, EPI_F32, EPI_GATE, EPI_RELU_DROP_BWD, EPI_F16_ACC, EPI_GELU_DROP, \
    EPI_GELU_DROP_BWD = range(9)
F16 = torch.float16


_DEV = [None]


def _dev():
    if _DEV[0] is None:
        _DEV[0] = torch.cuda.current_device()
    return _DEV[0]


def _s():
# ... 296 lines not shown
        dx = scratch[dxo[0]:dxo[0] + 2 * R * d].view(F16).view(R, d)
        dxd = scratch[dxo[1]:dxo[1] + 2 * R * d].view(F16).view(R, d) if sk else dx
        return dx, dxd


class ConvCall:

    _sizes = {}

    def __init__(self, ks, couts, weights, biases, gweights, gbiases, dgrad_weights):
        a = _lib.ConvArgs()
        a.nlayers = len(ks)
        for i, k in enumerate(ks):
            a.k[i], a.cout[i] = k, couts[i]
            a.w[i], a.b[i] = weights[i].data_ptr(), biases[i].data_ptr()
            a.g_w[i], a.g_b[i] = gweights[i].data_ptr(), gbiases[i].data_ptr()
        self.a = a
        self.dgrad_weights = dgrad_weights
        self.wt_of = None

    def _bind_wt(self):
        wt = TransposedWeights.active
        if wt is self.wt_of:
            return
        for i, W in self.dgrad_weights.items():
            img = wt.get(W, wait=False) if wt is not None else None
            self.a.wt[i] = 0 if img is None else img.data_ptr()
        self.wt_of = wt

    def sizes(self, a=None):
        a = self.a if a is None else a
        key = (a.B, a.T, a.C, a.nlayers, tuple(a.k), tuple(a.cout))
        s = ConvCall._sizes.get(key)
        if s is None:
            out_off, nb, sb, dxo = ctypes.c_int64(), ctypes.c_int64(), ctypes.c_int64(), ctypes.c_int64()
            mw, sw = ctypes.c_int64(), ctypes.c_int64()
            call("mms2ut_conv1d_glu_arena", ctypes.byref(a), ctypes.byref(out_off), ctypes.byref(nb))
            call("mms2ut_conv1d_glu_scratch", ctypes.byref(a), ctypes.byref(dxo), ctypes.byref(sb))
            call("mms2ut_conv1d_glu_ws", ctypes.byref(a), ctypes.byref(mw), ctypes.byref(sw))
            s = (nb.value, out_off.value, sb.value, mw.value, sw.value)
            ConvCall._sizes[key] = s
        return s

    def fwd(self, x, B, T, C):
        a = self.a
        a.B, a.T, a.C = B, T, C
        a.x = x.data_ptr()
        self._bind_wt()
        nb, out_off, _, mw, _ = self.sizes()
        arena = torch.empty(nb, dtype=torch.uint8, device=x.device)
        a.saved = arena.data_ptr()
        ws = stream_workspace(mw, x.device)
        call("mms2ut_conv1d_glu_fwd", ctypes.byref(a), None if ws is None else ws.data_ptr(), mw, _s())
        Tout = T
        for i in range(a.nlayers):
            Tout = (Tout - 1) // 2 + 1
        Cg = a.cout[a.nlayers - 1] // 2
        out = arena[out_off:out_off + 2 * B * Tout * Cg].view(F16).view(B * Tout, Cg)
        return arena, out, bytes(a)

    def bwd(self, snap, arena, dy):
        nb, _, sbytes, mw, sw = self.sizes(_lib.ConvArgs.from_buffer_copy(snap))
        dev = dy.device
        scratch = torch.empty(sbytes, dtype=torch.uint8, device=dev)
        if TransposedWeights.active is not None:
            TransposedWeights.active.wait_ready()
        main_ws = stream_workspace(mw, dev)
        side = 0
        if _Side.enabled:
            side_stream(dev)
            side = _Side.ptr
            with _SIDE_REGION:
                side_ws = _workspace("slab", sw, dev) if sw > 0 else None
        else:
            side_ws = _workspace("slab", sw, dev) if sw > 0 else None
        call("mms2ut_conv1d_glu_bwd", snap, dy.data_ptr(), scratch.data_ptr(),
             None if main_ws is None else main_ws.data_ptr(), mw, None if side_ws is None else side_ws.data_ptr(), sw,
             SIDE_WGRAD_BLOCKS if side else 0, _s(), side)
        if side:
            _Side.keep.extend((arena, scratch, dy))
            _Side.used = True


class FusionCall:

    _sizes = {}

    def __init__(self, flags, params, grads, dgrad_weights):
        a = _lib.FusionArgs()
        for f, v in flags.items():
            setattr(a, f, v)
        for f, t in params.items():
            setattr(a, f, 0 if t is None else t.data_ptr())
        for f, t in grads.items():
            setattr(a, f, 0 if t is None else t.data_ptr())
        self.a = a
        self.dgrad_weights = dgrad_weights
        self.wt_of = None

    def _bind_wt(self):
        wt = TransposedWeights.active
        if wt is self.wt_of:
            return
        for f, W in self.dgrad_weights.items():
            img = wt.get(W, wait=False) if wt is not None else None
            setattr(self.a, f, 0 if img is None else img.data_ptr())
        self.wt_of = wt

    def sizes(self, want_dimg, a=None):
        a = self.a if a is None else a
        key = (a.B, a.Te, a.Ti, a.Di, a.d, a.extra, a.gate, a.image_pre_norm, a.p_img > 0, a.p_txt > 0, a.p_attn > 0,
               bool(want_dimg))
        s = FusionCall._sizes.get(key)
        if s is None:
            oo, nb, sb, mw, sw = (ctypes.c_int64() for _ in range(5))
            so = (ctypes.c_int64 * 2)()
            call("mms2ut_gated_fusion_arena", ctypes.byref(a), ctypes.byref(oo), ctypes.byref(nb))
            call("mms2ut_gated_fusion_scratch", ctypes.byref(a), int(want_dimg), so, ctypes.byref(sb))
            call("mms2ut_gated_fusion_ws", ctypes.byref(a), ctypes.byref(mw), ctypes.byref(sw))
            s = (nb.value, oo.value, sb.value, list(so), mw.value, sw.value)
            FusionCall._sizes[key] = s
        return s

    def fwd(self, text, img, key_mask, B, Te, Ti, p, drops):
        a = self.a
        a.B, a.Te, a.Ti = B, Te, Ti
        a.p_img, a.p_txt, a.p_attn = p
        seeds = [dr[0] for dr in drops if dr is not None]
        a.seed = seeds[0] if seeds else 0
        assert all(sd == a.seed for sd in seeds), "one dropout seed per step"
        a.off_img, a.off_txt, a.off_attn = (dr[1] if dr is not None else 0 for dr in drops)
        a.key_mask, a.ld_mask = (key_mask.data_ptr(), key_mask.stride(0)) if key_mask is not None else (0, 0)
        a.text, a.img = text.data_ptr(), img.data_ptr()
        self._bind_wt()
        nb, oo, _, _, mw, _ = self.sizes(False)
        arena = torch.empty(nb, dtype=torch.uint8, device=text.device)
        a.saved = arena.data_ptr()
        ws = stream_workspace(mw, text.device)
        call("mms2ut_gated_fusion_fwd", ctypes.byref(a), None if ws is None else ws.data_ptr(), mw, _s())
        out = arena[oo:oo + 2 * B * Te * a.d].view(F16).view(B * Te, a.d)
        return arena, out, bytes(a)

    def bwd(self, snap, arena, keep, dres, want_dimg=False):
        a = _lib.FusionArgs.from_buffer_copy(snap)
        _, _, sbytes, so, mw, sw = self.sizes(want_dimg, a)
        dev = dres.device
        scratch = torch.empty(sbytes, dtype=torch.uint8, device=dev)
        if TransposedWeights.active is not None:
            TransposedWeights.active.wait_ready()
        main_ws = stream_workspace(mw, dev)
        side = 0
        if _Side.enabled:
            side_stream(dev)
            side = _Side.ptr
            with _SIDE_REGION:
                side_ws = _workspace("slab", sw, dev) if sw > 0 else None
        else:
            side_ws = _workspace("slab", sw, dev) if sw > 0 else None
        call("mms2ut_gated_fusion_bwd", snap, dres.data_ptr(), int(want_dimg), scratch.data_ptr(),
             None if main_ws is None else main_ws.data_ptr(), mw, None if side_ws is None else side_ws.data_ptr(), sw,
             SIDE_WGRAD_BLOCKS if side else 0, _s(), side)
        if side:
            _Side.keep.extend((arena, scratch, dres) + tuple(keep))
            _Side.used = True
        R, d = a.B * a.Te, a.d
        dtext = scratch[so[0]:so[0] + 2 * R * d].view(F16).view(R, d)
        if not want_dimg:
            return dtext
        Ri = a.B * a.Ti
        return dtext, scratch[so[1]:so[1] + 2 * Ri * a.Di].view(F16).view(Ri, a.Di)


def linear_dgrad(dy, W, out=None, *, epi=EPI_F16, aux=None, p=0.0, accumulate=False, drop=None):
    M, N = dy.shape
    K = W.shape[1]
    if out is None:
        out = torch.empty(M, K, dtype=F16, device=dy.device)
    if accumulate:
        epi = EPI_F16_ACC
    seed, off = drop if (drop is not None and p > 0) else (0, 0)
    WT = TransposedWeights.active.get(W) if TransposedWeights.active is not None else None
    if WT is not None:
        gemm(dy, WT, out, M, K, N, a_kc=True, b_kc=True, lda=dy.stride(0), ldb=WT.stride(0),
             ldc=out.stride(0), epi=epi, aux=aux, ldaux=(aux.stride(0) if aux is not None else 0), p=p,
             seed=seed, offset=off, ld_rng=K)
        return out
    gemm(dy, W, out, M, K, N, a_kc=True, b_kc=False, lda=dy.stride(0), ldb=W.stride(0),
         ldc=out.stride(0), epi=epi, aux=aux, ldaux=(aux.stride(0) if aux is not None else 0), p=p,
         seed=seed, offset=off, ld_rng=K)
    return out


def _splitk_for(tiles, kred, slots=512):
    s = max(1, min(16, slots // max(tiles, 1)))
    while s > 1 and kred // s < 256:
# ... 206 lines not shown
    M, N = dy.shape
    L = _lib.load()
    ctx = side_begin(dy) if side else None
    with (ctx or _NULLCTX):
        nparts = L.mms2ut_colsum_nparts(M)
        part = _workspace("colsum", nparts * N, dy.device)
        call("mms2ut_colsum_f16", dy.data_ptr(), M, N, dy.stride(0), part.data_ptr(), nparts, _s())
        call("mms2ut_colsum_parts", part.data_ptr(), nparts, N, db.data_ptr(), int(accumulate), _s())
    return db



def layernorm(x, g, b, eps=1e-5, *, out=None, grp=0, grp_out=0, p=0.0, drop=None):
    R, D = x.shape
    mean = torch.empty(R, dtype=torch.float32, device=x.device)
    rstd = torch.empty(R, dtype=torch.float32, device=x.device)
    if out is None and not grp and p == 0.0:
        y = torch.empty_like(x)
        call("mms2ut_layernorm_fwd", x.data_ptr(), g.data_ptr(), b.data_ptr(), y.data_ptr(),
             mean.data_ptr(), rstd.data_ptr(), R, D, eps, _s())
        return y, mean, rstd
    y = torch.empty_like(x) if out is None else out
    assert y.is_contiguous() and y.shape[-1] == D
    seed, off = drop if p > 0 else (0, 0)
    call("mms2ut_layernorm_fwd_ex", x.data_ptr(), g.data_ptr(), b.data_ptr(), y.data_ptr(),
         mean.data_ptr(), rstd.data_ptr(), R, D, eps, int(grp), int(grp_out), float(p), seed, off, _s())
    return y, mean, rstd


def layernorm_bwd(dy, x, g, mean, rstd, dgb, dres=None, want_dx=True, emit=None, dy_grp=0, dy_grp_out=0,
                  dy_p=0.0, dy_drop=None, dgb_accumulate=False):
    R, D = x.shape
    if dy_grp or dy_p > 0:
        assert emit is None and D % 256 == 0 and D <= 1024
        L = _lib.load()
        nparts = L.mms2ut_layernorm_bwd_nparts(R, D)
        part = torch.empty(nparts, 2 * D, dtype=torch.float32, device=x.device)
        dx = torch.empty_like(x) if want_dx else None
        seed, off = dy_drop if dy_p > 0 else (0, 0)
        call("mms2ut_layernorm_bwd_ex", dy.data_ptr(), x.data_ptr(), g.data_ptr(), mean.data_ptr(),
             rstd.data_ptr(), _p(dres), _p(dx), part.data_ptr(), R, D, None, 0.0, 0, 0, int(dy_grp),
             int(dy_grp_out), float(dy_p), seed, off, _s())
        ctx = side_begin(part)
        with (ctx or _NULLCTX):
            call("mms2ut_colsum_parts", part.data_ptr(), nparts, 2 * D, dgb.data_ptr(), 0, _s())
        return dx
    L = _lib.load()
    nparts = L.mms2ut_layernorm_bwd_nparts(R, D)
    part = torch.empty(nparts, 2 * D, dtype=torch.float32, device=x.device)
    dx = torch.empty_like(x) if want_dx else None
    dxd, p, seed, off = None, 0.0, 0, 0
    if emit is not None and emit[0] > 0:
        p, (seed, off) = emit
        dxd = torch.empty_like(x)
    call("mms2ut_layernorm_bwd", dy.data_ptr(), x.data_ptr(), g.data_ptr(), mean.data_ptr(),
         rstd.data_ptr(), _p(dres), _p(dx), part.data_ptr(), R, D, _p(dxd), float(p), seed, off, _s())
    ctx = side_begin(part)
    with (ctx or _NULLCTX):
        call("mms2ut_colsum_parts", part.data_ptr(), nparts, 2 * D, dgb.data_ptr(), int(dgb_accumulate), _s())
    if emit is not None:
        return dx, (dxd if dxd is not None else dx)
    return dx



def attn_softmax(S, Z, H, Tq, Tk, ldS, key_len=None, key_mask=None, causal=False, extra_key=False,
                 p=0.0, drop=None):
    P = torch.empty_like(S)
    Pd = torch.empty_like(S) if p > 0 else P
    seed, off = drop if p > 0 else (0, 0)
    call("mms2ut_attn_softmax_fwd", S.data_ptr(), P.data_ptr(), Pd.data_ptr(), Z, H, Tq, Tk, ldS,
         _p(key_len), _p(key_mask), (key_mask.stride(0) if key_mask is not None else 0),
         int(causal), int(extra_key), float(p), seed, off, _s())
    return P, Pd


def attn_softmax_bwd(P, dPd, Z, H, Tq, Tk, ldS, p=0.0, drop=None, out=None):
    seed, off = drop if p > 0 else (0, 0)
    dS = dPd if out is None else out
    call("mms2ut_attn_softmax_bwd", P.data_ptr(), dPd.data_ptr(), dS.data_ptr(), Z, H, Tq, Tk, ldS,
         None, 0, 0, float(p), seed, off, _s())
    return dS

FLASH_HD = (64, 96, 128)


def _attn_args(q, k, v, o, ldq, ldk, ldv, ldo, B, H, Tq, Tk, hd, scale, key_len, causal, p, drop, lse,
               sq=0, sk=0, sv=0, so=0):
    seed, off = drop if p > 0 else (0, 0)
    return _lib.ATTN_ARGS.pack(q.data_ptr(), k.data_ptr(), v.data_ptr(), o.data_ptr(), ldq, ldk, ldv, ldo,
                               sq, sk, sv, so, B, H, Tq, Tk, hd, 0 if key_len is None else key_len.data_ptr(),
                               int(causal), scale, p, seed, off, lse.data_ptr())


def mha_fwd(q, k, v, o, ldq, ldk, ldv, ldo, B, H, Tq, Tk, hd, scale, key_len=None, causal=False,
            p=0.0, drop=None, sq=0, sk=0, sv=0, so=0):
    lse = torch.empty(B * H * Tq, dtype=torch.float32, device=q.device)
    a = _attn_args(q, k, v, o, ldq, ldk, ldv, ldo, B, H, Tq, Tk, hd, scale, key_len, causal, p, drop, lse,
                   sq, sk, sv, so)
    call("mms2ut_mha_varlen_fwd", a, _s())
    return lse


def mha_bwd(q, k, v, o, ldq, ldk, ldv, ldo, B, H, Tq, Tk, hd, scale, key_len, causal, p, drop, lse,
            dout, lddo, dq, lddq, dk, lddk, dv, lddv):
    a = _attn_args(q, k, v, o, ldq, ldk, ldv, ldo, B, H, Tq, Tk, hd, scale, key_len, causal, p, drop, lse)
    Dd = torch.empty(B * H * Tq, dtype=torch.float32, device=q.device)
    call("mms2ut_mha_varlen_bwd", a, dout.data_ptr(), int(lddo), 0, Dd.data_ptr(), dq.data_ptr(),
         int(lddq), 0, dk.data_ptr(), int(lddk), 0, dv.data_ptr(), int(lddv), 0, _s())



def dropout(x, p, drop, out=None):
    out = x if out is None else out
    if p <= 0:
        if out.data_ptr() != x.data_ptr():
            out.copy_(x)
        return out
    seed, off = drop
    call("mms2ut_dropout_fwd", x.data_ptr(), out.data_ptr(), x.numel(), float(p), seed, off, _s())
    return out


def dropout_mask(n, p, seed, offset, device):
    m = torch.empty(n, dtype=torch.uint8, device=device)
    call("mms2ut_dropout_mask", m.data_ptr(), n, float(p), int(seed), int(offset), _s())
    return m


def encoder_embed(h, pos_table, lens32, B, T, D, scale, p, drop):
    x = torch.empty_like(h)
    seed, off = drop if p > 0 else (0, 0)
    call("mms2ut_encoder_embed_fwd", h.data_ptr(), pos_table.data_ptr(), lens32.data_ptr(),
         x.data_ptr(), B, T, D, float(scale), float(p), seed, off, _s())
    return x


def scale_dropout_bwd(dx, scale, p, drop, out=None):
    out = torch.empty_like(dx) if out is None else out
    seed, off = drop if p > 0 else (0, 0)
    call("mms2ut_scale_dropout_bwd", dx.data_ptr(), out.data_ptr(), dx.numel(), float(scale),
         float(p), seed, off, _s())
    return out


def token_embed(tok, E, pos_table, B, T, D, pad, scale, p, drop):
    x = torch.empty(B * T, D, dtype=F16, device=E.device)
    seed, off = drop if p > 0 else (0, 0)
    call("mms2ut_token_embed_fwd", tok.data_ptr(), E.data_ptr(), pos_table.data_ptr(), x.data_ptr(),
         B, T, D, pad, float(scale), float(p), seed, off, _s())
    return x


def token_embed_bwd(tok, dx, dE32, B, T, D, pad, scale, p, drop):
    seed, off = drop if p > 0 else (0, 0)
    call("mms2ut_token_embed_bwd", tok.data_ptr(), dx.data_ptr(), dE32.data_ptr(), B, T, D, dE32.shape[0], pad,
         float(scale), float(p), seed, off, _s())


def add_f32_to_f16(a, b32, out):
    call("mms2ut_add_f32_to_f16", a.data_ptr(), b32.data_ptr(), out.data_ptr(), a.numel(), _s())
    return out


def add_f16(a, b, out=None):
    out = torch.empty_like(a) if out is None else out
# ... 273 lines not shown
```

### multimodal-s2ut_amd/model.py

```python
import math
import os
import re
from collections import OrderedDict

import numpy as np
import torch

from . import kernels as K
from .kernels import F16, round_up



def default_cfg(**over):
    cfg = dict(
        input_feat_per_channel=80, input_channels=1, conv_kernel_sizes=(5, 5), conv_channels=1024,
        encoder_embed_dim=768, encoder_ffn_embed_dim=3072, encoder_layers=12,
        encoder_attention_heads=8, decoder_embed_dim=768, decoder_ffn_embed_dim=3072,
        decoder_layers=6, decoder_attention_heads=8, dropout=0.1, attention_dropout=0.1,
        activation_dropout=0.1, vocab_size=1004, padding_idx=1, eos=2, label_smoothing=0.2,
        fusion=True, multimodal_attention_type="multimodal_attention", use_selective_gate=True,
        image_feat_dim=768, image_pre_norm=True, SA_image_dropout=0.1, SA_text_dropout=0.0,
        SA_attention_dropout=0.1, modality_dropout=-0.5, audio_dropout=-0.5,
        max_source_positions=6000, max_target_positions=3000, no_scale_embedding=False,
        external_multimodal_transformer_layers=None,
# ... 862 lines not shown
        self._fusion[Di] = fc
        return fc

    def fusion_fwd(self, text, img, img_mask, B, Te):
        cfg = self.cfg
        d = cfg["encoder_embed_dim"]
        _, Ti, Di = img.shape
        extra = cfg["multimodal_attention_type"] == "multimodal_attention"
        Tk = Ti + 1 if extra else Ti
        pimg, ptxt, pat = self._p("SA_image_dropout"), self._p("SA_text_dropout"), self._p("SA_attention_dropout")
        drops = (self._drop(pimg, B * Ti * Di), self._drop(ptxt, B * Te * d), self._drop(pat, B * Te * Tk))
        img2 = img.reshape(B * Ti, Di).contiguous()
        text = text.contiguous()
        arena, out, snap = self._fusion_call(Di).fwd(text, img2, img_mask, B, Te, Ti, (pimg, ptxt, pat), drops)
        c = {"B": B, "Te": Te, "Ti": Ti, "Di": Di, "Tk": Tk, "extra": extra, "pimg": pimg, "ptxt": ptxt, "pat": pat,
             "drop_img": drops[0], "drop_txt": drops[1], "drop_attn": drops[2], "arena": arena, "snap": snap,
             "keep": tuple(t for t in (text, img2, img_mask) if t is not None)}
        return out, c

    def fusion_bwd(self, c, dres, want_dimg=False):
        return self._fusion_call(c["Di"]).bwd(c["snap"], c["arena"], c["keep"], dres.contiguous(), want_dimg)

    def fusion_fwd_ref(self, text, img, img_mask, B, Te):
        cfg = self.cfg
        d = cfg["encoder_embed_dim"]
        _, Ti, Di = img.shape
        att = cfg["multimodal_attention_type"]
        extra = att == "multimodal_attention"
        Tk = Ti + 1 if extra else Ti
        c = {"B": B, "Te": Te, "Ti": Ti, "Di": Di, "Tk": Tk, "extra": extra}
        img2 = img.reshape(B * Ti, Di)
        pimg = self._p("SA_image_dropout")
        c["drop_img"] = self._drop(pimg, B * Ti * Di)
        c["ln_fused"] = cfg["image_pre_norm"] and Di % 256 == 0 and Di <= 1024
        if c["ln_fused"]:
            imgd = torch.empty(B, Tk, Di, dtype=F16, device=img.device)
            if extra:
                imgd[:, Ti:].zero_()
            _, c["im"], c["ir"] = K.layernorm(img2, self.P("encoder.image_pre_norm_module.weight"),
                                              self.P("encoder.image_pre_norm_module.bias"), out=imgd,
                                              grp=Ti if extra else 0, grp_out=Tk if extra else 0, p=pimg,
                                              drop=c["drop_img"])
            c["img_in"] = img2
            imgd = imgd.view(B * Tk, Di)
        else:
            if cfg["image_pre_norm"]:
                imgn, c["im"], c["ir"] = K.layernorm(img2, self.P("encoder.image_pre_norm_module.weight"),
                                                     self.P("encoder.image_pre_norm_module.bias"))
                c["img_in"] = img2
            else:
                imgn = img2
            if pimg > 0:
                imgn = K.dropout(imgn, pimg, c["drop_img"])
            if extra:
                imgd = torch.zeros(B, Tk, Di, dtype=F16, device=img.device)
                K.copy2d(imgn.view(B, Ti * Di), imgd.view(B, Tk * Di), B, Ti * Di)
                imgd = imgd.view(B * Tk, Di)
            else:
                imgd = imgn
        c["imgd"] = imgd
        ptxt = self._p("SA_text_dropout")
        c["drop_txt"] = self._drop(ptxt, B * Te * d)
        textd = K.dropout(text, ptxt, c["drop_txt"], out=torch.empty_like(text)) if ptxt > 0 else text
        c["textd"] = textd
        if extra:
            pre = "encoder.multimodal_attns.0"
            if Di == d:
                W = self.P(pre + ".in_proj_weight")
                Wq, Wkv = W[:d], W[d:]
            else:
                Wq = self.P(pre + ".q_proj_weight")
                Wkv = self.params.span(pre + ".k_proj_weight", pre + ".v_proj_weight").view(2 * d, Di)
            bias = self.P(pre + ".in_proj_bias")
            bq, bkv = bias[:d], bias[d:]
            Wo, bo = self.P(pre + ".out_proj.weight"), self.P(pre + ".out_proj.bias")
        else:
            pre = "encoder.selective_attns.0"
            Wq, bq = self.P(pre + ".q_proj.weight"), self.P(pre + ".q_proj.bias")
            Wkv = self.params.span(pre + ".k_proj.weight", pre + ".v_proj.weight").view(2 * d, Di)
            bkv = self.params.span(pre + ".k_proj.bias", pre + ".v_proj.bias")
            Wo, bo = self.P(pre + ".proj.weight"), self.P(pre + ".proj.bias")
        c["pre"] = pre
        q = K.linear(textd, Wq, bq)
        kv = K.linear(imgd, Wkv, bkv)
        if extra:
            bkv_rows = self.params.span(pre + ".bias_k", pre + ".bias_v").view(1, 2 * d)
            K.copy2d(bkv_rows.expand(B, 2 * d), kv.view(B, Tk * 2 * d)[:, Ti * 2 * d:], B, 2 * d)
        c["q"], c["kv"] = q, kv
        key_mask = img_mask
        c["key_mask"] = key_mask
        pat = self._p("SA_attention_dropout")
        c["drop_attn"] = self._drop(pat, B * Te * Tk)
        O = torch.empty(B * Te, d, dtype=F16, device=text.device)
        c["P"], c["Pd"], c["ldS"] = attn_fwd(q, kv, kv[:, d:], d, 2 * d, 2 * d, B, 1, Te, Tk, d,
                                             d ** -0.5, O, d, key_mask=key_mask, extra_key=extra,
                                             p=pat, drop=c["drop_attn"])
        c["O"], c["pat"], c["pimg"], c["ptxt"] = O, pat, pimg, ptxt
        if cfg["use_selective_gate"]:
            merge = torch.empty(B * Te, 2 * d, dtype=F16, device=text.device)
            K.linear(O, Wo, bo, out=merge[:, :d], ldc=2 * d)
            K.copy2d(textd, merge[:, d:], B * Te, d)
            g = torch.empty(B * Te, d, dtype=F16, device=text.device)
            res = K.linear(merge, self.P("encoder.gate_denses.0.weight"), self.P("encoder.gate_denses.0.bias"),
                           epi=K.EPI_GATE, aux=merge, out2=g)
            c["merge"], c["g"] = merge, g
        else:
            res = K.linear(O, Wo, bo, epi=K.EPI_DROP_RESID, aux=textd)
        return res, c

    def fusion_bwd_ref(self, c, dres, want_dimg=False):
        cfg = self.cfg
        d = cfg["encoder_embed_dim"]
        B, Te, Ti, Di, Tk, extra, pre = c["B"], c["Te"], c["Ti"], c["Di"], c["Tk"], c["extra"], c["pre"]
        if extra:
            if Di == d:
                W = self.P(pre + ".in_proj_weight")
                Wq, Wkv = W[:d], W[d:]
                gW = self.G(pre + ".in_proj_weight")
                gWq, gWkv = gW[:d], gW[d:]
            else:
                Wq = self.P(pre + ".q_proj_weight")
                Wkv = self.params.span(pre + ".k_proj_weight", pre + ".v_proj_weight").view(2 * d, Di)
                gWq = self.G(pre + ".q_proj_weight")
                gWkv = self.params.span(pre + ".k_proj_weight", pre + ".v_proj_weight", grad=True).view(2 * d, Di)
            gb = self.G(pre + ".in_proj_bias")
            gbq, gbkv = gb[:d], gb[d:]
            Wo, gWo, gbo = self.P(pre + ".out_proj.weight"), self.G(pre + ".out_proj.weight"), self.G(pre + ".out_proj.bias")
        else:
            Wq, gWq, gbq = self.P(pre + ".q_proj.weight"), self.G(pre + ".q_proj.weight"), self.G(pre + ".q_proj.bias")
            Wkv = self.params.span(pre + ".k_proj.weight", pre + ".v_proj.weight").view(2 * d, Di)
            gWkv = self.params.span(pre + ".k_proj.weight", pre + ".v_proj.weight", grad=True).view(2 * d, Di)
            gbkv = self.params.span(pre + ".k_proj.bias", pre + ".v_proj.bias", grad=True)
            Wo, gWo, gbo = self.P(pre + ".proj.weight"), self.G(pre + ".proj.weight"), self.G(pre + ".proj.bias")
        if cfg["use_selective_gate"]:
            dpre, dmerge = K.gate_bwd(dres, c["merge"], c["g"])
            K.linear_wgrad(dpre, c["merge"], self.G("encoder.gate_denses.0.weight"),
                           db=self.G("encoder.gate_denses.0.bias"))
            K.linear_dgrad(dpre, self.P("encoder.gate_denses.0.weight"), out=dmerge, accumulate=True)
            dOp = dmerge[:, :d]
            dtext = dmerge[:, d:]
        else:
            dOp = dres
            dtext = dres
        K.linear_wgrad(dOp, c["O"], gWo,
                       db=gbo)
        dO = K.linear_dgrad(dOp, Wo)
        q, kv = c["q"], c["kv"]
        dq = torch.empty_like(q)
        dkv = torch.empty_like(kv)
        attn_bwd(dO, d, q, kv, kv[:, d:], d, 2 * d, 2 * d, c["P"], c["Pd"], c["ldS"], B, 1, Te, Tk, d,
                 d ** -0.5, dq, dkv, dkv[:, d:], d, 2 * d, 2 * d, p=c["pat"], drop=c["drop_attn"])
        if extra:
            rows = dkv.view(B, Tk * 2 * d)[:, Ti * 2 * d:]
            K.bias_grad(rows, self.params.span(pre + ".bias_k", pre + ".bias_v", grad=True), side=False)
            rows.zero_()
        K.linear_wgrad(dkv, c["imgd"], gWkv,
                       db=gbkv)
        dimg_in = None
        if c["ln_fused"]:
            dimgd = K.linear_dgrad(dkv, Wkv)
            dimg_in = K.layernorm_bwd(dimgd, c["img_in"], self.P("encoder.image_pre_norm_module.weight"), c["im"],
                                      c["ir"], self.params.span("encoder.image_pre_norm_module.weight",
                                                                "encoder.image_pre_norm_module.bias", grad=True),
                                      want_dx=want_dimg, dy_grp=Ti if extra else 0, dy_grp_out=Tk if extra else 0,
                                      dy_p=c["pimg"], dy_drop=c["drop_img"])
        elif cfg["image_pre_norm"] or want_dimg:
            dimgd = K.linear_dgrad(dkv, Wkv)
            if extra:
                dimg = torch.empty(B * Ti, Di, dtype=F16, device=dkv.device)
                K.copy2d(dimgd.view(B, Tk * Di), dimg.view(B, Ti * Di), B, Ti * Di)
            else:
                dimg = dimgd
            if c["pimg"] > 0:
                dimg = K.dropout(dimg, c["pimg"], c["drop_img"])
            if cfg["image_pre_norm"]:
                dimg_in = K.layernorm_bwd(dimg, c["img_in"], self.P("encoder.image_pre_norm_module.weight"), c["im"],
                                          c["ir"], self.params.span("encoder.image_pre_norm_module.weight",
                                                                    "encoder.image_pre_norm_module.bias", grad=True),
                                          want_dx=want_dimg)
            else:
                dimg_in = dimg
        K.linear_wgrad(dq, c["textd"], gWq,
                       db=gbq)
        dtext_total = torch.empty(B * Te, d, dtype=F16, device=dres.device)
        K.copy2d(dtext, dtext_total, B * Te, d)
        K.linear_dgrad(dq, Wq, out=dtext_total, accumulate=True)
        if c["ptxt"] > 0:
            dtext_total = K.dropout(dtext_total, c["ptxt"], c["drop_txt"])
        if want_dimg:
            return dtext_total, dimg_in
        return dtext_total

    def _mha_w(self, p, d, kdim, grad=False):
        b = (self.G if grad else self.P)(p + ".in_proj_bias")
        if kdim == d:
            W = (self.G if grad else self.P)(p + ".in_proj_weight")
            return W[:d], W[d:], b[:d], b[d:]
        return ((self.G if grad else self.P)(p + ".q_proj_weight"),
                self.params.span(p + ".k_proj_weight", p + ".v_proj_weight", grad=grad).view(2 * d, kdim), b[:d], b[d:])

    def mml_fwd(self, p, x, mem2, B, Tq, Tm, d, kdim, H, pp, sa_first=True, self_len=None, mem_len=None,
                mem_km=None):
        hd = d // H
        R = B * Tq
        dev = x.device
        c = {"x": x, "pp": pp, "B": B, "Te": Tq, "Ti": Tm, "img2": mem2, "d": d, "kdim": kdim, "H": H, "p": p,
             "sa_first": sa_first}

        def sa_block(xin):
            qkv = K.linear(xin, self.P(p + ".self_attn.in_proj_weight"), self.P(p + ".self_attn.in_proj_bias"))
            O = torch.empty(R, d, dtype=F16, device=dev)
            c["drop_sa"] = self._drop(pp, B * H * Tq * Tq)
            c["sattn"] = attn_forward(qkv, qkv[:, d:], qkv[:, 2 * d:], 3 * d, 3 * d, 3 * d, B, H, Tq, Tq, hd,
                                      hd ** -0.5, O, d, key_len=self_len, p=pp, drop=c["drop_sa"])
            c["qkv"], c["sO"], c["sa_in"] = qkv, O, xin
            c["drop1"] = self._drop(pp, R * d)
            y1 = K.linear(O, self.P(p + ".self_attn.out_proj.weight"), self.P(p + ".self_attn.out_proj.bias"),
                          epi=K.EPI_DROP_RESID, aux=xin, p=pp, drop=c["drop1"])
            x1, c["m1"], c["r1"] = K.layernorm(y1, self.P(p + ".norm1.weight"), self.P(p + ".norm1.bias"))
            c["y1"], c["x1"] = y1, x1
            return x1

        def ca_block(xin):
            Wq, Wkv, bq, bkv = self._mha_w(p + ".multihead_attn", d, kdim)
            q = K.linear(xin, Wq, bq)
            kv = K.linear(mem2, Wkv, bkv)
            O2 = torch.empty(R, d, dtype=F16, device=dev)
            c["drop_ca"] = self._drop(pp, B * H * Tq * Tm)
            c["cattn"] = attn_forward(q, kv, kv[:, d:], d, 2 * d, 2 * d, B, H, Tq, Tm, hd, hd ** -0.5, O2, d,
                                      key_len=mem_len, key_mask=mem_km, p=pp, drop=c["drop_ca"])
            c["q"], c["kv"], c["cO"], c["ca_in"] = q, kv, O2, xin
            c["drop2"] = self._drop(pp, R * d)
            y2 = K.linear(O2, self.P(p + ".multihead_attn.out_proj.weight"), self.P(p + ".multihead_attn.out_proj.bias"),
                          epi=K.EPI_DROP_RESID, aux=xin, p=pp, drop=c["drop2"])
            x2, c["m2"], c["r2"] = K.layernorm(y2, self.P(p + ".norm2.weight"), self.P(p + ".norm2.bias"))
            c["y2"], c["x2"] = y2, x2
            return x2

        xa = ca_block(sa_block(x)) if sa_first else sa_block(ca_block(x))
        F_ = self.P(p + ".linear1.weight").shape[0]
        c["ff_in"] = xa
        c["drop_act"] = self._drop(pp, R * F_)
        z = torch.empty(R, F_, dtype=F16, device=dev)
        h = K.linear(xa, self.P(p + ".linear1.weight"), self.P(p + ".linear1.bias"), epi=K.EPI_GELU_DROP, out2=z,
                     p=pp, drop=c["drop_act"])
        c["z"], c["h"] = z, h
        c["drop3"] = self._drop(pp, R * d)
        y3 = K.linear(h, self.P(p + ".linear2.weight"), self.P(p + ".linear2.bias"), epi=K.EPI_DROP_RESID, aux=xa,
                      p=pp, drop=c["drop3"])
        x3, c["m3"], c["r3"] = K.layernorm(y3, self.P(p + ".norm3.weight"), self.P(p + ".norm3.bias"))
        c["y3"] = y3
        return x3, c
# ... 469 lines not shown
```

Before: 1.966 million audio-frames/s.

## Add query-side reassociation route for gated-fusion image attention

Adds an alternative gated-fusion attention path that folds the K/V projection weights into the query side. Scores are computed as (q·Wk_aug)·img and the output as (P·img)·Wv_aug, so the per-image-token K/V projection is no longer materialized. A FLOP-based heuristic picks this route when Te·Dia·d work is smaller than Tk·Di·2d work, and an override knob is exposed. New softmax kernels handle the bias/extra-key augmented columns, and pack/unpack kernels build the augmented weights and scatter their gradients. The backward pass is rewritten the same way, which means more batched GEMMs over Di-wide operands and extra scratch buffers.

```diff
diff --git a/include/mms2ut.h b/include/mms2ut.h
--- a/include/mms2ut.h
+++ b/include/mms2ut.h
@@ -135,6 +135,19 @@
                             int H, int Tq, int Tk, int64_t ldS, const int32_t* key_len, int causal,
                             int extra_key, float p, uint64_t seed, uint64_t offset,
                             hipStream_t stream);
+int mms2ut_attn_softmax_fwd_aug(const mms2ut_half* S, mms2ut_half* P, mms2ut_half* Pd, int Z, int Tq, int Tk,
+                                int64_t ldS, const uint8_t* key_mask, int64_t ld_mask, int extra_key, float p,
+                                uint64_t seed, uint64_t offset, const mms2ut_half* q_aug, int64_t ld_q,
+                                float scale, int n_img, mms2ut_half* u_aug, int64_t ld_u, int npad,
+                                hipStream_t stream);
+int mms2ut_attn_softmax_bwd_aug(const mms2ut_half* P, const mms2ut_half* dPd, mms2ut_half* dS, int Z, int Tq,
+                                int Tk, int64_t ldS, float p, uint64_t seed, uint64_t offset,
+                                const mms2ut_half* du_aug, int64_t ld_du, float scale, int n_img,
+                                mms2ut_half* dq_aug, int64_t ld_dq, int npad, hipStream_t stream);
+int mms2ut_fusion_pack_kv(const mms2ut_half* wkv, const mms2ut_half* bkv, const mms2ut_half* bias_kv,
+                          mms2ut_half* out, int rows, int Di, int Dia, hipStream_t stream);
+int mms2ut_fusion_unpack_kv(const mms2ut_half* dw, mms2ut_half* g_wkv, mms2ut_half* g_bkv,
+                            mms2ut_half* g_bias_kv, int rows, int Di, int Dia, hipStream_t stream);
 
 typedef struct mms2ut_attn_args {
   const mms2ut_half* q;
@@ -347,6 +360,7 @@
                           int64_t main_ws_floats, float* side_ws, int64_t side_ws_floats, int side_blocks,
                           hipStream_t main, hipStream_t side);
 
+int mms2ut_gated_fusion_set_route(int mode);
 typedef struct mms2ut_gated_fusion {
   int B, Te, Ti, Di, d;
   int extra;
@@ -364,6 +378,7 @@
   const mms2ut_half* img;
   void* saved;
 } mms2ut_gated_fusion;
+int mms2ut_gated_fusion_route(const mms2ut_gated_fusion* f);
 int mms2ut_gated_fusion_arena(const mms2ut_gated_fusion* f, int64_t* out_offset, int64_t* bytes);
 int mms2ut_gated_fusion_scratch(const mms2ut_gated_fusion* f, int want_dimg, int64_t* offsets, int64_t* bytes);
 int mms2ut_gated_fusion_ws(const mms2ut_gated_fusion* f, int64_t* main_floats, int64_t* side_floats);
diff --git a/multimodal-s2ut_amd/_lib.py b/multimodal-s2ut_amd/_lib.py
--- a/multimodal-s2ut_amd/_lib.py
+++ b/multimodal-s2ut_amd/_lib.py
@@ -164,6 +164,12 @@
                                       f32, u64, u64, vp]),
     "mms2ut_attn_softmax_bwd": (i32, [vp, vp, vp, i32, i32, i32, i32, i64, vp, i32, i32, f32, u64,
                                       u64, vp]),
+    "mms2ut_attn_softmax_fwd_aug": (i32, [vp, vp, vp, i32, i32, i32, i64, vp, i64, i32, f32, u64, u64,
+                                          vp, i64, f32, i32, vp, i64, i32, vp]),
+    "mms2ut_attn_softmax_bwd_aug": (i32, [vp, vp, vp, i32, i32, i32, i64, f32, u64, u64, vp, i64, f32, i32,
+                                          vp, i64, i32, vp]),
+    "mms2ut_fusion_pack_kv": (i32, [vp, vp, vp, vp, i32, i32, i32, vp]),
+    "mms2ut_fusion_unpack_kv": (i32, [vp, vp, vp, vp, i32, i32, i32, vp]),
     "mms2ut_mha_varlen_fwd": (i32, [vp, vp]),
     "mms2ut_mha_varlen_bwd": (i32, [vp, vp, i64, i64, vp, vp, i64, i64, vp, i64, i64,
                                     vp, i64, i64, vp]),
@@ -203,6 +209,8 @@
     "mms2ut_layer_ws": (i32, [vp, vp, vp]),
     "mms2ut_layer_fwd": (i32, [vp, vp, i64, vp]),
     "mms2ut_layer_bwd": (i32, [vp, vp, vp, vp]),
+    "mms2ut_gated_fusion_set_route": (i32, [i32]),
+    "mms2ut_gated_fusion_route": (i32, [vp]),
     "mms2ut_gated_fusion_arena": (i32, [vp, vp, vp]),
     "mms2ut_gated_fusion_scratch": (i32, [vp, i32, vp, vp]),
     "mms2ut_gated_fusion_ws": (i32, [vp, vp, vp]),
diff --git a/multimodal-s2ut_amd/csrc/layers.hip b/multimodal-s2ut_amd/csrc/layers.hip
--- a/multimodal-s2ut_amd/csrc/layers.hip
+++ b/multimodal-s2ut_amd/csrc/layers.hip
@@ -666,9 +666,19 @@
 }
 
 struct FusDims {
-  int64_t B, Te, Ti, Tk, Di, d, Rt, Ri, Rk, ldS;
-  bool extra, gate, pre, ln_fused;
+  int64_t B, Te, Ti, Tk, Di, Dia, d, Rt, Ri, Rk, ldS;
+  bool extra, gate, pre, ln_fused, qs;
 };
+
+int g_fus_route = -1;
+
+bool fus_query_side(int64_t B, int64_t Te, int64_t Tk, int64_t Di, int64_t Dia, int64_t d, bool pre) {
+  if (g_fus_route >= 0) return g_fus_route == 1;
+  const int64_t nx = pre ? 1 : 0;
+  const int64_t key = (2 + nx) * B * Tk * Di * 2 * d + 6 * B * Te * Tk * d;
+  const int64_t qry = 6 * B * Te * Dia * d + (4 + 2 * nx) * B * Te * Tk * Di;
+  return qry < key;
+}
 
 FusDims fus_dims(const mms2ut_gated_fusion* f) {
   FusDims D;
@@ -678,10 +688,13 @@
   D.Rt = D.B * D.Te; D.Ri = D.B * D.Ti; D.Rk = D.B * D.Tk;
   D.ldS = (D.Tk + 7) / 8 * 8;
   D.ln_fused = D.pre && D.Di % 256 == 0 && D.Di <= 1024;
+  D.Dia = (D.Di + 2 + 63) / 64 * 64;
+  D.qs = fus_query_side(D.B, D.Te, D.Tk, D.Di, D.Dia, D.d, D.pre);
   return D;
 }
 
-enum { FA_IM = 0, FA_IR, FA_IMGN, FA_IMGD, FA_TEXTD, FA_Q, FA_KV, FA_S, FA_P, FA_PD, FA_O, FA_MERGE, FA_G, FA_OUT, FA_N };
+enum { FA_IM = 0, FA_IR, FA_IMGN, FA_IMGD, FA_TEXTD, FA_Q, FA_KV, FA_WAUG, FA_QK, FA_U, FA_S, FA_P, FA_PD, FA_O, FA_MERGE,
+       FA_G, FA_OUT, FA_N };
 void fus_arena_sizes(const mms2ut_gated_fusion* f, const FusDims& D, int64_t* sz) {
   for (int i = 0; i < FA_N; ++i) sz[i] = 0;
   const int64_t h = 2;
@@ -690,7 +703,12 @@
   if (D.ln_fused || D.extra) sz[FA_IMGD] = D.Rk * D.Di * h;
   if (f->p_txt > 0.f) sz[FA_TEXTD] = D.Rt * D.d * h;
   sz[FA_Q] = D.Rt * D.d * h;
-  sz[FA_KV] = D.Rk * 2 * D.d * h;
+  if (D.qs) {
+    sz[FA_WAUG] = 2 * D.d * D.Dia * h;
+    sz[FA_QK] = sz[FA_U] = D.Rt * D.Dia * h;
+  } else {
+    sz[FA_KV] = D.Rk * 2 * D.d * h;
+  }
   sz[FA_S] = sz[FA_P] = D.Rt * D.ldS * h;
   if (f->p_attn > 0.f) sz[FA_PD] = sz[FA_P];
   sz[FA_O] = D.Rt * D.d * h;
@@ -698,14 +716,19 @@
   sz[FA_OUT] = D.Rt * D.d * h;
 }
 
-enum { FS_DPRE = 0, FS_DMERGE, FS_DO, FS_DQ, FS_DKV, FS_DPD, FS_DIMGD, FS_DIMG, FS_DIMGIN, FS_DTEXT, FS_LNP, FS_KVP,
-       FS_BPART, FS_N };
+enum { FS_DPRE = 0, FS_DMERGE, FS_DO, FS_DQ, FS_DKV, FS_DU, FS_DQK, FS_DWAUG, FS_DPD, FS_DIMGD, FS_DIMG, FS_DIMGIN, FS_DTEXT,
+       FS_LNP, FS_KVP, FS_BPART, FS_N };
 void fus_scratch_sizes(const mms2ut_gated_fusion* f, const FusDims& D, int want_dimg, int64_t* sz) {
   for (int i = 0; i < FS_N; ++i) sz[i] = 0;
   const int64_t h = 2;
   if (D.gate) { sz[FS_DPRE] = D.Rt * D.d * h; sz[FS_DMERGE] = D.Rt * 2 * D.d * h; }
   sz[FS_DO] = sz[FS_DQ] = D.Rt * D.d * h;
-  sz[FS_DKV] = D.Rk * 2 * D.d * h;
+  if (D.qs) {
+    sz[FS_DU] = sz[FS_DQK] = D.Rt * D.Dia * h;
+    sz[FS_DWAUG] = 2 * D.d * D.Dia * h;
+  } else {
+    sz[FS_DKV] = D.Rk * 2 * D.d * h;
+  }
   sz[FS_DPD] = D.Rt * D.ldS * h;
   if (D.pre || want_dimg) {
     sz[FS_DIMGD] = D.Rk * D.Di * h;
@@ -714,7 +737,7 @@
     if (D.pre) sz[FS_LNP] = (int64_t)mms2ut_layernorm_bwd_nparts(D.Ri, (int)D.Di) * 2 * D.Di * 4;
   }
   sz[FS_DTEXT] = D.Rt * D.d * h;
-  if (D.extra) sz[FS_KVP] = (int64_t)mms2ut_colsum_nparts(D.B) * 2 * D.d * 4;
+  if (D.extra && !D.qs) sz[FS_KVP] = (int64_t)mms2ut_colsum_nparts(D.B) * 2 * D.d * 4;
   sz[FS_BPART] = (int64_t)mms2ut_colsum_nparts(std::max(D.Rt, D.Rk)) * 2 * D.d * 4;
 }
 
@@ -747,6 +770,17 @@
   return mms2ut_copy2d_pad(nullptr, 0, p, pitch_elems, rows, 0, (int)width_elems, s);
 }
 
+}
+
+extern "C" int mms2ut_gated_fusion_set_route(int mode) {
+  MMS_REQUIRE(mode >= -1 && mode <= 1, "gated_fusion_set_route: mode must be -1, 0 or 1 (got %d)", mode);
+  g_fus_route = mode;
+  return 0;
+}
+
+extern "C" int mms2ut_gated_fusion_route(const mms2ut_gated_fusion* f) {
+  if (fus_check(f)) return -1;
+  return fus_dims(f).qs ? 1 : 0;
 }
 
 extern "C" int mms2ut_gated_fusion_arena(const mms2ut_gated_fusion* f, int64_t* out_offset, int64_t* bytes) {
@@ -788,9 +822,16 @@
     sw = std::max(sw, (int64_t)s * N * K + (int64_t)s * N);
   };
   const int64_t d = D.d;
-  fw(D.Rt, d, d); fw(D.Rk, 2 * d, D.Di); fw(D.Rt, d, d); fw(D.Rt, d, 2 * d);
-  fw(D.Rt, 2 * d, d); fw(D.Rt, d, d); fw(D.Rk, D.Di, 2 * d); fw(D.Rt, d, d);
-  ww(D.Rt, d, 2 * d); ww(D.Rt, d, d); ww(D.Rk, 2 * d, D.Di); ww(D.Rt, d, d);
+  fw(D.Rt, d, d); fw(D.Rt, d, d); fw(D.Rt, d, 2 * d);
+  fw(D.Rt, 2 * d, d); fw(D.Rt, d, d); fw(D.Rt, d, d);
+  ww(D.Rt, d, 2 * d); ww(D.Rt, d, d); ww(D.Rt, d, d);
+  if (D.qs) {
+    fw(D.Rt, D.Dia, d); fw(D.Rt, d, D.Dia);
+    ww(D.Rt, d, D.Dia);
+  } else {
+    fw(D.Rk, 2 * d, D.Di); fw(D.Rk, D.Di, 2 * d);
+    ww(D.Rk, 2 * d, D.Di);
+  }
   *main_floats = mw;
   *side_floats = sw;
   return 0;
@@ -843,21 +884,38 @@
   }
   mms2ut_half *q = H_(FA_Q), *kv = H_(FA_KV), *O = H_(FA_O);
   if ((rc = linear(c, textd, f->wq, f->bq, q, D.Rt, d, d))) return rc;
-  if ((rc = linear(c, imgd, f->wkv, f->bkv, kv, D.Rk, 2 * d, Di))) return rc;
-  if (D.extra && (rc = mms2ut_copy2d(f->bias_kv, 0, kv + D.Ti * 2 * d, D.Tk * 2 * d, D.B, (int)(2 * d), s))) return rc;
   const float scale = (float)pow((double)d, -0.5);
   mms2ut_half *S = H_(FA_S), *P = H_(FA_P), *Pd = f->p_attn > 0.f ? H_(FA_PD) : P;
-  {
+  if (D.qs) {
+    const int64_t Dia = D.Dia;
+    mms2ut_half *waug = H_(FA_WAUG), *qk = H_(FA_QK), *U = H_(FA_U);
+    if ((rc = mms2ut_fusion_pack_kv(f->wkv, f->bkv, D.extra ? f->bias_kv : nullptr, waug, (int)(2 * d), (int)Di,
+                                    (int)Dia, s))) return rc;
+    if ((rc = gemm_nt(c, q, d, waug, Dia, 0, qk, Dia, D.Rt, Dia, d, MMS_EPI_F16, nullptr, nullptr, 0, 0.f, 0, 0, Dia)))
+      return rc;
+    mms2ut_gemm_args a = batched(qk, imgd, S, (int)D.Te, (int)D.Tk, (int)Di, 1, 1, Dia, Di, D.ldS, (int)D.B, D.Te * Dia,
+                                 D.Tk * Di, D.Te * D.ldS, scale);
+    if ((rc = mms2ut_gemm_f16(&a, s))) return rc;
+    if ((rc = mms2ut_attn_softmax_fwd_aug(S, P, Pd, (int)D.B, (int)D.Te, (int)D.Tk, D.ldS, f->key_mask,
+                                          f->key_mask ? f->ld_mask : 0, D.extra ? 1 : 0, f->p_attn,
+                                          f->p_attn > 0.f ? f->seed : 0, f->p_attn > 0.f ? f->off_attn : 0, qk + Di, Dia,
+                                          scale, (int)D.Ti, U + Di, Dia, (int)(Dia - Di), s))) return rc;
+    a = batched(Pd, imgd, U, (int)D.Te, (int)Di, (int)D.Tk, 1, 0, D.ldS, Di, Dia, (int)D.B, D.Te * D.ldS, D.Tk * Di,
+                D.Te * Dia, 1.f);
+    if ((rc = mms2ut_gemm_f16(&a, s))) return rc;
+    if ((rc = gemm_nt(c, U, Dia, waug + d * Dia, Dia, 1, O, d, D.Rt, d, Dia, MMS_EPI_F16, nullptr, nullptr, 0, 0.f, 0, 0,
+                      d))) return rc;
+  } else {
+    if ((rc = linear(c, imgd, f->wkv, f->bkv, kv, D.Rk, 2 * d, Di))) return rc;
+    if (D.extra && (rc = mms2ut_copy2d(f->bias_kv, 0, kv + D.Ti * 2 * d, D.Tk * 2 * d, D.B, (int)(2 * d), s))) return rc;
     mms2ut_gemm_args a = batched(q, kv, S, (int)D.Te, (int)D.Tk, (int)d, 1, 1, d, 2 * d, D.ldS, (int)D.B, D.Te * d,
                                  D.Tk * 2 * d, D.Te * D.ldS, scale);
     if ((rc = mms2ut_gemm_f16(&a, s))) return rc;
-  }
-  if ((rc = mms2ut_attn_softmax_fwd(S, P, Pd, (int)D.B, 1, (int)D.Te, (int)D.Tk, D.ldS, nullptr, f->key_mask,
-                                    f->key_mask ? f->ld_mask : 0, 0, D.extra ? 1 : 0, f->p_attn,
-                                    f->p_attn > 0.f ? f->seed : 0, f->p_attn > 0.f ? f->off_attn : 0, s))) return rc;
-  {
-    mms2ut_gemm_args a = batched(Pd, kv + d, O, (int)D.Te, (int)d, (int)D.Tk, 1, 0, D.ldS, 2 * d, d, (int)D.B,
-                                 D.Te * D.ldS, D.Tk * 2 * d, D.Te * d, 1.f);
+    if ((rc = mms2ut_attn_softmax_fwd(S, P, Pd, (int)D.B, 1, (int)D.Te, (int)D.Tk, D.ldS, nullptr, f->key_mask,
+                                      f->key_mask ? f->ld_mask : 0, 0, D.extra ? 1 : 0, f->p_attn,
+                                      f->p_attn > 0.f ? f->seed : 0, f->p_attn > 0.f ? f->off_attn : 0, s))) return rc;
+    a = batched(Pd, kv + d, O, (int)D.Te, (int)d, (int)D.Tk, 1, 0, D.ldS, 2 * d, d, (int)D.B, D.Te * D.ldS, D.Tk * 2 * d,
+                D.Te * d, 1.f);
     if ((rc = mms2ut_gemm_f16(&a, s))) return rc;
   }
   mms2ut_half* out = H_(FA_OUT);
@@ -923,31 +981,57 @@
   mms2ut_half *dq = SH(FS_DQ), *dkv = SH(FS_DKV), *dPd = SH(FS_DPD);
   const int B = (int)D.B, Te = (int)D.Te, Tk = (int)D.Tk;
   const int64_t sS = D.Te * D.ldS;
-  {
+  if (D.qs) {
+    const int64_t Dia = D.Dia;
+    const mms2ut_half *waug = H_(FA_WAUG), *qk = H_(FA_QK), *U = H_(FA_U);
+    mms2ut_half *dU = SH(FS_DU), *dqk = SH(FS_DQK), *dwa = SH(FS_DWAUG);
+    if ((rc = gemm_nt(c, dO, d, waug + d * Dia, Dia, 0, dU, Dia, D.Rt, Dia, d, MMS_EPI_F16, nullptr, nullptr, 0, 0.f, 0, 0,
+                      Dia))) return rc;
+    if ((rc = wgrad_auto(c, dO, d, U, Dia, dwa + d * Dia, nullptr, D.Rt, d, Dia, side_blocks))) return rc;
+    mms2ut_gemm_args a = batched(dU, imgd, dPd, Te, Tk, (int)Di, 1, 1, Dia, Di, D.ldS, B, D.Te * Dia, D.Tk * Di, sS, 1.f);
+    if ((rc = mms2ut_gemm_f16(&a, main))) return rc;
+    if ((rc = mms2ut_attn_softmax_bwd_aug(P, dPd, dPd, B, Te, Tk, D.ldS, f->p_attn, f->p_attn > 0.f ? f->seed : 0,
+                                          f->p_attn > 0.f ? f->off_attn : 0, dU + Di, Dia, scale, (int)D.Ti, dqk + Di,
+                                          Dia, (int)(Dia - Di), main))) return rc;
+    a = batched(dPd, imgd, dqk, Te, (int)Di, Tk, 1, 0, D.ldS, Di, Dia, B, sS, D.Tk * Di, D.Te * Dia, scale);
+    if ((rc = mms2ut_gemm_f16(&a, main))) return rc;
+    if ((rc = wgrad_auto(c, q, d, dqk, Dia, dwa, nullptr, D.Rt, d, Dia, side_blocks))) return rc;
+    if ((rc = fork(c)) ||
+        (rc = mms2ut_fusion_unpack_kv(dwa, f->g_wkv, f->g_bkv, D.extra ? f->g_bias_kv : nullptr, (int)(2 * d), (int)Di,
+                                      (int)Dia, side))) return rc;
+    if ((rc = gemm_nt(c, dqk, Dia, waug, Dia, 1, dq, d, D.Rt, d, Dia, MMS_EPI_F16, nullptr, nullptr, 0, 0.f, 0, 0, d)))
+      return rc;
+    if (D.pre || want_dimg) {
+      mms2ut_half* dimgd = SH(FS_DIMGD);
+      a = batched(dPd, qk, dimgd, Tk, (int)Di, Te, 0, 0, D.ldS, Dia, Di, B, sS, D.Te * Dia, D.Tk * Di, scale);
+      if ((rc = mms2ut_gemm_f16(&a, main))) return rc;
+      a = batched(Pd, dU, dimgd, Tk, (int)Di, Te, 0, 0, D.ldS, Dia, Di, B, sS, D.Te * Dia, D.Tk * Di, 1.f);
+      a.epi = MMS_EPI_F16_ACC;
+      if ((rc = mms2ut_gemm_f16(&a, main))) return rc;
+    }
+  } else {
     mms2ut_gemm_args a = batched(dO, kv + d, dPd, Te, Tk, (int)d, 1, 1, d, 2 * d, D.ldS, B, D.Te * d, D.Tk * 2 * d, sS, 1.f);
     if ((rc = mms2ut_gemm_f16(&a, main))) return rc;
     a = batched(Pd, dO, dkv + d, Tk, (int)d, Te, 0, 0, D.ldS, d, 2 * d, B, sS, D.Te * d, D.Tk * 2 * d, 1.f);
     if ((rc = mms2ut_gemm_f16(&a, main))) return rc;
-  }
-  if ((rc = mms2ut_attn_softmax_bwd(P, dPd, dPd, B, 1, Te, Tk, D.ldS, nullptr, 0, 0, f->p_attn,
-                                    f->p_attn > 0.f ? f->seed : 0, f->p_attn > 0.f ? f->off_attn : 0, main))) return rc;
-  {
-    mms2ut_gemm_args a = batched(dPd, kv, dq, Te, (int)d, Tk, 1, 0, D.ldS, 2 * d, d, B, sS, D.Tk * 2 * d, D.Te * d, scale);
+    if ((rc = mms2ut_attn_softmax_bwd(P, dPd, dPd, B, 1, Te, Tk, D.ldS, nullptr, 0, 0, f->p_attn,
+                                      f->p_attn > 0.f ? f->seed : 0, f->p_attn > 0.f ? f->off_attn : 0, main))) return rc;
+    a = batched(dPd, kv, dq, Te, (int)d, Tk, 1, 0, D.ldS, 2 * d, d, B, sS, D.Tk * 2 * d, D.Te * d, scale);
     if ((rc = mms2ut_gemm_f16(&a, main))) return rc;
     a = batched(dPd, q, dkv, Tk, (int)d, Te, 0, 0, D.ldS, d, 2 * d, B, sS, D.Te * d, D.Tk * 2 * d, scale);
     if ((rc = mms2ut_gemm_f16(&a, main))) return rc;
-  }
-  if (D.extra) {
-    mms2ut_half* rows = dkv + D.Ti * 2 * d;
-    const int np = mms2ut_colsum_nparts(D.B);
-    if ((rc = mms2ut_colsum_f16(rows, D.B, (int)(2 * d), D.Tk * 2 * d, SF(FS_KVP), np, main))) return rc;
-    if ((rc = mms2ut_colsum_parts(SF(FS_KVP), np, (int)(2 * d), f->g_bias_kv, 0, main))) return rc;
-    if ((rc = zero_rows(rows, D.Tk * 2 * d, 2 * d, D.B, main))) return rc;
-  }
-  if ((rc = wgrad_auto(c, dkv, 2 * d, imgd, Di, f->g_wkv, f->g_bkv, D.Rk, 2 * d, Di, side_blocks))) return rc;
+    if (D.extra) {
+      mms2ut_half* rows = dkv + D.Ti * 2 * d;
+      const int np = mms2ut_colsum_nparts(D.B);
+      if ((rc = mms2ut_colsum_f16(rows, D.B, (int)(2 * d), D.Tk * 2 * d, SF(FS_KVP), np, main))) return rc;
+      if ((rc = mms2ut_colsum_parts(SF(FS_KVP), np, (int)(2 * d), f->g_bias_kv, 0, main))) return rc;
+      if ((rc = zero_rows(rows, D.Tk * 2 * d, 2 * d, D.B, main))) return rc;
+    }
+    if ((rc = wgrad_auto(c, dkv, 2 * d, imgd, Di, f->g_wkv, f->g_bkv, D.Rk, 2 * d, Di, side_blocks))) return rc;
+  }
   if (D.ln_fused) {
     mms2ut_half* dimgd = SH(FS_DIMGD);
-    if ((rc = dgrad(c, dkv, 2 * d, f->wkv, f->wt_kv, dimgd, D.Rk, 2 * d, Di))) return rc;
+    if (!D.qs && (rc = dgrad(c, dkv, 2 * d, f->wkv, f->wt_kv, dimgd, D.Rk, 2 * d, Di))) return rc;
     if ((rc = mms2ut_layernorm_bwd_ex(dimgd, f->img, f->ln_g, at<float>(A, off, FA_IM), at<float>(A, off, FA_IR), nullptr,
                                       want_dimg ? SH(FS_DIMGIN) : nullptr, SF(FS_LNP), D.Ri, (int)Di, nullptr, 0.f, 0, 0,
                                       D.extra ? D.Ti : 0, D.extra ? D.Tk : 0, f->p_img, f->p_img > 0.f ? f->seed : 0,
@@ -957,7 +1041,7 @@
       return rc;
   } else if (D.pre || want_dimg) {
     mms2ut_half* dimgd = SH(FS_DIMGD);
-    if ((rc = dgrad(c, dkv, 2 * d, f->wkv, f->wt_kv, dimgd, D.Rk, 2 * d, Di))) return rc;
+    if (!D.qs && (rc = dgrad(c, dkv, 2 * d, f->wkv, f->wt_kv, dimgd, D.Rk, 2 * d, Di))) return rc;
     mms2ut_half* dimg = dimgd;
     if (D.extra) {
       dimg = SH(FS_DIMG);
diff --git a/multimodal-s2ut_amd/csrc/ops.hip b/multimodal-s2ut_amd/csrc/ops.hip
--- a/multimodal-s2ut_amd/csrc/ops.hip
+++ b/multimodal-s2ut_amd/csrc/ops.hip
@@ -432,6 +432,15 @@
   }
 }
 
+struct SoftmaxAug {
+  const h16* in;
+  long ld_in;
+  h16* out;
+  long ld_out;
+  int n_img, npad;
+  float scale;
+};
+
 MMS_DEV bool key_valid(int j, int i, int Tk, int klen, const uint8_t* km, int causal, int extra_key) {
   if (j >= Tk) return false;
   if (extra_key && j == Tk - 1) return true;
@@ -447,12 +456,17 @@
                                                           long ldS, const int* __restrict__ key_len,
                                                           const uint8_t* __restrict__ key_mask, long ld_mask,
                                                           int causal, int extra_key, float p, uint32_t thresh,
-                                                          uint64_t seed, uint64_t offset) {
+                                                          uint64_t seed, uint64_t offset, SoftmaxAug aug) {
   if (thresh) seed = mms_step_seed(seed);
   const int lane = threadIdx.x & 63;
   const long row = (long)blockIdx.x * 4 + (threadIdx.x >> 6);
   if (row >= (long)Z * Tq) return;
   const int z = (int)(row / Tq), i = (int)(row % Tq);
+  float add0 = 0.f, add1 = 0.f;
+  if (aug.in) {
+    add0 = aug.scale * (float)aug.in[row * aug.ld_in];
+    add1 = aug.scale * (float)aug.in[row * aug.ld_in + 1];
+  }
   const int b = z / H;
   const int klen = key_len ? key_len[b] : Tk;
   const uint8_t* km = key_mask ? key_mask + (long)b * ld_mask : nullptr;
@@ -467,7 +481,8 @@
 #pragma unroll
       for (int e = 0; e < 4; ++e) {
         const int j = j0 + e;
-        v[c][e] = key_valid(j, i, Tk, klen, km, causal, extra_key) ? (float)t[e] : -INFINITY;
+        v[c][e] = key_valid(j, i, Tk, klen, km, causal, extra_key)
+                      ? (float)t[e] + (aug.in ? (j < aug.n_img ? add0 : add1) : 0.f) : -INFINITY;
         mx = fmaxf(mx, v[c][e]);
       }
     } else {
@@ -490,6 +505,7 @@
   const float ds = thresh ? 1.f / (1.f - p) : 1.f;
   h16* pr = P + row * ldS;
   h16* pdr = Pd + row * ldS;
+  float r_img = 0.f, r_ext = 0.f;
 #pragma unroll
   for (int c = 0; c < CPL; ++c) {
     const int j0 = (lane + c * 64) * 4;
@@ -503,10 +519,18 @@
           const bool keep = mms_keep(seed, offset + (uint64_t)row * Tk + (j0 + e), thresh);
           od[e] = keep ? o[e] * ds : 0.f;
         }
+        if (aug.out) {
+          if (j0 + e < aug.n_img) r_img += od[e]; else r_ext += od[e];
+        }
       }
       st4(pr + j0, o[0], o[1], o[2], o[3]);
       if (thresh) st4(pdr + j0, od[0], od[1], od[2], od[3]);
     }
+  }
+  if (aug.out) {
+    r_img = wave_sum(r_img);
+    r_ext = wave_sum(r_ext);
+    if (lane < aug.npad) aug.out[row * aug.ld_out + lane] = (h16)(lane == 0 ? r_img : lane == 1 ? r_ext : 0.f);
   }
 }
 
@@ -514,12 +538,17 @@
 __global__ void __launch_bounds__(256) softmax_bwd_kernel(const h16* __restrict__ P, const h16* __restrict__ dPd,
                                                           h16* __restrict__ dS, int Z, int H, int Tq, int Tk,
                                                           long ldS, float p, uint32_t thresh, uint64_t seed,
-                                                          uint64_t offset) {
+                                                          uint64_t offset, SoftmaxAug aug) {
   if (thresh) seed = mms_step_seed(seed);
   const int lane = threadIdx.x & 63;
   const long row = (long)blockIdx.x * 4 + (threadIdx.x >> 6);
   if (row >= (long)Z * Tq) return;
   const float ds = thresh ? 1.f / (1.f - p) : 1.f;
+  float add0 = 0.f, add1 = 0.f;
+  if (aug.in) {
+    add0 = (float)aug.in[row * aug.ld_in];
+    add1 = (float)aug.in[row * aug.ld_in + 1];
+  }
   float pv[CPL][4], gv[CPL][4];
   float s = 0.f;
 #pragma unroll
@@ -533,7 +562,7 @@
         float m = ds;
         if (thresh && j < Tk) m = mms_keep(seed, offset + (uint64_t)row * Tk + j, thresh) ? ds : 0.f;
         pv[c][e] = (j < Tk) ? (float)a[e] : 0.f;
-        gv[c][e] = (j < Tk) ? (float)g[e] * m : 0.f;
+        gv[c][e] = (j < Tk) ? ((float)g[e] + (aug.in ? (j < aug.n_img ? add0 : add1) : 0.f)) * m : 0.f;
         s += pv[c][e] * gv[c][e];
       }
     } else {
@@ -542,17 +571,55 @@
     }
   }
   s = wave_sum(s);
+  float t_img = 0.f, t_ext = 0.f;
 #pragma unroll
   for (int c = 0; c < CPL; ++c) {
     const int j0 = (lane + c * 64) * 4;
     if (j0 < Tk) {
       float o[4];
 #pragma unroll
-      for (int e = 0; e < 4; ++e) o[e] = pv[c][e] * (gv[c][e] - s);
+      for (int e = 0; e < 4; ++e) {
+        o[e] = pv[c][e] * (gv[c][e] - s);
+        if (aug.out) {
+          if (j0 + e < aug.n_img) t_img += o[e]; else t_ext += o[e];
+        }
+      }
       st4(dS + row * ldS + j0, o[0], o[1], o[2], o[3]);
     }
   }
+  if (aug.out) {
+    t_img = wave_sum(t_img);
+    t_ext = wave_sum(t_ext);
+    if (lane < aug.npad)
+      aug.out[row * aug.ld_out + lane] = (h16)(lane == 0 ? aug.scale * t_img : lane == 1 ? aug.scale * t_ext : 0.f);
+  }
   (void)Z; (void)H;
+}
+
+__global__ void fusion_pack_kv_kernel(const h16* __restrict__ wkv, const h16* __restrict__ bkv,
+                                      const h16* __restrict__ bias_kv, h16* __restrict__ out, int rows, int Di,
+                                      int Dia) {
+  const long n = (long)rows * Dia;
+  for (long t = blockIdx.x * (long)blockDim.x + threadIdx.x; t < n; t += (long)gridDim.x * blockDim.x) {
+    const int r = (int)(t / Dia), i = (int)(t % Dia);
+    h16 v = (h16)0.f;
+    if (i < Di) v = wkv[(long)r * Di + i];
+    else if (i == Di) v = bkv[r];
+    else if (i == Di + 1 && bias_kv) v = bias_kv[r];
+    out[t] = v;
+  }
+}
+
+__global__ void fusion_unpack_kv_kernel(const h16* __restrict__ dw, h16* __restrict__ g_wkv, h16* __restrict__ g_bkv,
+                                        h16* __restrict__ g_bias_kv, int rows, int Di, int Dia) {
+  const long n = (long)rows * Dia;
+  for (long t = blockIdx.x * (long)blockDim.x + threadIdx.x; t < n; t += (long)gridDim.x * blockDim.x) {
+    const int r = (int)(t / Dia), i = (int)(t % Dia);
+    const h16 v = dw[t];
+    if (i < Di) g_wkv[(long)r * Di + i] = v;
+    else if (i == Di) g_bkv[r] = v;
+    else if (i == Di + 1 && g_bias_kv) g_bias_kv[r] = v;
+  }
 }
 
 __global__ void dropout_kernel(const h16* __restrict__ x, h16* __restrict__ y, long n, float p,
@@ -1029,10 +1096,10 @@
   return mms::check_launch("colsum_f16");
 }
 
-extern "C" int mms2ut_attn_softmax_fwd(const h16* S, h16* P, h16* Pd, int Z, int H, int Tq, int Tk,
-                                       int64_t ldS, const int32_t* key_len, const uint8_t* key_mask,
-                                       int64_t ld_mask, int causal, int extra_key,
-                                       float p, uint64_t seed, uint64_t offset, hipStream_t s) {
+static int softmax_fwd_launch(const h16* S, h16* P, h16* Pd, int Z, int H, int Tq, int Tk, int64_t ldS,
+                              const int32_t* key_len, const uint8_t* key_mask, int64_t ld_mask, int causal,
+                              int extra_key, float p, uint64_t seed, uint64_t offset, const SoftmaxAug& aug,
+                              hipStream_t s) {
   MMS_REQUIRE(ldS % 4 == 0 && ldS >= Tk, "softmax: ldS must be a multiple of 4 and >= Tk");
   MMS_REQUIRE(p < 1.f, "softmax: p must be < 1");
   const long rows = (long)Z * Tq;
@@ -1041,8 +1108,44 @@
   return pick_cpl((Tk + 3) / 4, [&](auto C) {
     hipLaunchKernelGGL((softmax_fwd_kernel<decltype(C)::value>), dim3((rows + 3) / 4), dim3(256), 0, s,
                        S, P, Pd, Z, H, Tq, Tk, (long)ldS, key_len, key_mask, (long)ld_mask, causal,
-                       extra_key, p, th, seed, offset);
+                       extra_key, p, th, seed, offset, aug);
     return mms::check_launch("attn_softmax_fwd");
+  });
+}
+
+extern "C" int mms2ut_attn_softmax_fwd(const h16* S, h16* P, h16* Pd, int Z, int H, int Tq, int Tk,
+                                       int64_t ldS, const int32_t* key_len, const uint8_t* key_mask,
+                                       int64_t ld_mask, int causal, int extra_key,
+                                       float p, uint64_t seed, uint64_t offset, hipStream_t s) {
+  return softmax_fwd_launch(S, P, Pd, Z, H, Tq, Tk, ldS, key_len, key_mask, ld_mask, causal, extra_key, p, seed,
+                            offset, SoftmaxAug{}, s);
+}
+
+static bool aug_ok(const h16* in, int64_t ld_in, const h16* out, int64_t ld_out, int n_img, int npad, int Tk) {
+  return in && out && ld_in >= 2 && ld_out >= npad && npad >= 2 && npad <= 64 && n_img >= 0 && n_img <= Tk;
+}
+
+extern "C" int mms2ut_attn_softmax_fwd_aug(const h16* S, h16* P, h16* Pd, int Z, int Tq, int Tk, int64_t ldS,
+                                           const uint8_t* key_mask, int64_t ld_mask, int extra_key, float p,
+                                           uint64_t seed, uint64_t offset, const h16* q_aug, int64_t ld_q,
+                                           float scale, int n_img, h16* u_aug, int64_t ld_u, int npad,
+                                           hipStream_t s) {
+  MMS_REQUIRE(aug_ok(q_aug, ld_q, u_aug, ld_u, n_img, npad, Tk), "softmax_fwd_aug: bad augmentation columns");
+  const SoftmaxAug aug{q_aug, (long)ld_q, u_aug, (long)ld_u, n_img, npad, scale};
+  return softmax_fwd_launch(S, P, Pd, Z, 1, Tq, Tk, ldS, nullptr, key_mask, ld_mask, 0, extra_key, p, seed, offset,
+                            aug, s);
+}
+
+static int softmax_bwd_launch(const h16* P, const h16* dPd, h16* dS, int Z, int H, int Tq, int Tk, int64_t ldS,
+                              float p, uint64_t seed, uint64_t offset, const SoftmaxAug& aug, hipStream_t s) {
+  MMS_REQUIRE(ldS % 4 == 0 && ldS >= Tk, "softmax_bwd: ldS must be a multiple of 4 and >= Tk");
+  const long rows = (long)Z * Tq;
+  if (rows == 0) return 0;
+  const uint32_t th = mms_drop_thresh(p);
+  return pick_cpl((Tk + 3) / 4, [&](auto C) {
+    hipLaunchKernelGGL((softmax_bwd_kernel<decltype(C)::value>), dim3((rows + 3) / 4), dim3(256), 0, s,
+                       P, dPd, dS, Z, H, Tq, Tk, (long)ldS, p, th, seed, offset, aug);
+    return mms::check_launch("attn_softmax_bwd");
   });
 }
 
@@ -1050,16 +1153,37 @@
                                        int Tk, int64_t ldS, const int32_t* key_len, int causal,
                                        int extra_key, float p, uint64_t seed, uint64_t offset,
                                        hipStream_t s) {
-  MMS_REQUIRE(ldS % 4 == 0 && ldS >= Tk, "softmax_bwd: ldS must be a multiple of 4 and >= Tk");
-  const long rows = (long)Z * Tq;
-  if (rows == 0) return 0;
-  const uint32_t th = mms_drop_thresh(p);
   (void)key_len; (void)causal; (void)extra_key;
-  return pick_cpl((Tk + 3) / 4, [&](auto C) {
-    hipLaunchKernelGGL((softmax_bwd_kernel<decltype(C)::value>), dim3((rows + 3) / 4), dim3(256), 0, s,
-                       P, dPd, dS, Z, H, Tq, Tk, (long)ldS, p, th, seed, offset);
-    return mms::check_launch("attn_softmax_bwd");
-  });
+  return softmax_bwd_launch(P, dPd, dS, Z, H, Tq, Tk, ldS, p, seed, offset, SoftmaxAug{}, s);
+}
+
+extern "C" int mms2ut_attn_softmax_bwd_aug(const h16* P, const h16* dPd, h16* dS, int Z, int Tq, int Tk,
+                                           int64_t ldS, float p, uint64_t seed, uint64_t offset, const h16* du_aug,
+                                           int64_t ld_du, float scale, int n_img, h16* dq_aug, int64_t ld_dq,
+                                           int npad, hipStream_t s) {
+  MMS_REQUIRE(aug_ok(du_aug, ld_du, dq_aug, ld_dq, n_img, npad, Tk), "softmax_bwd_aug: bad augmentation columns");
+  const SoftmaxAug aug{du_aug, (long)ld_du, dq_aug, (long)ld_dq, n_img, npad, scale};
+  return softmax_bwd_launch(P, dPd, dS, Z, 1, Tq, Tk, ldS, p, seed, offset, aug, s);
+}
+
+extern "C" int mms2ut_fusion_pack_kv(const h16* wkv, const h16* bkv, const h16* bias_kv, h16* out, int rows,
+                                     int Di, int Dia, hipStream_t s) {
+  MMS_REQUIRE(wkv && bkv && out && rows > 0 && Di > 0 && Dia >= Di + 2, "fusion_pack_kv: bad arguments");
+  const long n = (long)rows * Dia;
+  const long nb = (n + 255) / 256;
+  hipLaunchKernelGGL(fusion_pack_kv_kernel, dim3((unsigned)(nb < 2048 ? nb : 2048)), dim3(256), 0, s,
+                     wkv, bkv, bias_kv, out, rows, Di, Dia);
+  return mms::check_launch("fusion_pack_kv");
+}
+
+extern "C" int mms2ut_fusion_unpack_kv(const h16* dw, h16* g_wkv, h16* g_bkv, h16* g_bias_kv, int rows, int Di,
+                                       int Dia, hipStream_t s) {
+  MMS_REQUIRE(dw && g_wkv && g_bkv && rows > 0 && Di > 0 && Dia >= Di + 2, "fusion_unpack_kv: bad arguments");
+  const long n = (long)rows * Dia;
+  const long nb = (n + 255) / 256;
+  hipLaunchKernelGGL(fusion_unpack_kv_kernel, dim3((unsigned)(nb < 2048 ? nb : 2048)), dim3(256), 0, s,
+                     dw, g_wkv, g_bkv, g_bias_kv, rows, Di, Dia);
+  return mms::check_launch("fusion_unpack_kv");
 }
 
 extern "C" int mms2ut_dropout_fwd(const h16* x, h16* y, int64_t n, float p, uint64_t seed,
diff --git a/multimodal-s2ut_amd/kernels.py b/multimodal-s2ut_amd/kernels.py
--- a/multimodal-s2ut_amd/kernels.py
+++ b/multimodal-s2ut_amd/kernels.py
@@ -402,6 +402,34 @@
             _Side.used = True
 
 
+def fusion_route(a):
+    r = _lib.load().mms2ut_gated_fusion_route(ctypes.byref(a))
+    if r < 0:
+        raise RuntimeError("mms2ut_gated_fusion_route: " + _lib.load().mms2ut_last_error().decode())
+    return r
+
+
+def fusion_set_route(mode):
+    call("mms2ut_gated_fusion_set_route", int(mode))
+
+
+def fusion_pack_kv(Wkv, bkv, bias_kv, Dia):
+    rows, Di = Wkv.shape
+    assert Wkv.is_contiguous() and bkv.is_contiguous() and (bias_kv is None or bias_kv.is_contiguous())
+    out = torch.empty(rows, Dia, dtype=F16, device=Wkv.device)
+    call("mms2ut_fusion_pack_kv", Wkv.data_ptr(), bkv.data_ptr(), _p(bias_kv), out.data_ptr(), rows, Di, Dia, _s())
+    return out
+
+
+def fusion_unpack_kv(dw, gWkv, gbkv, g_bias_kv):
+    rows, Di = gWkv.shape
+    assert gWkv.is_contiguous() and gbkv.is_contiguous() and dw.is_contiguous()
+    ctx = side_begin(dw)
+    with (ctx or _NULLCTX):
+        call("mms2ut_fusion_unpack_kv", dw.data_ptr(), gWkv.data_ptr(), gbkv.data_ptr(), _p(g_bias_kv), rows, Di,
+             dw.shape[1], _s())
+
+
 class FusionCall:
 
     _sizes = {}
@@ -427,10 +455,15 @@
             setattr(self.a, f, 0 if img is None else img.data_ptr())
         self.wt_of = wt
 
+    def route(self, B, Te, Ti):
+        a = self.a
+        a.B, a.Te, a.Ti = B, Te, Ti
+        return fusion_route(a)
+
     def sizes(self, want_dimg, a=None):
         a = self.a if a is None else a
         key = (a.B, a.Te, a.Ti, a.Di, a.d, a.extra, a.gate, a.image_pre_norm, a.p_img > 0, a.p_txt > 0, a.p_attn > 0,
-               bool(want_dimg))
+               bool(want_dimg), fusion_route(a))
         s = FusionCall._sizes.get(key)
         if s is None:
             oo, nb, sb, mw, sw = (ctypes.c_int64() for _ in range(5))
@@ -803,6 +836,25 @@
          None, 0, 0, float(p), seed, off, _s())
     return dS
 
+def attn_softmax_aug(S, Z, Tq, Tk, ldS, q_aug, scale, n_img, u_aug, npad, key_mask=None, extra_key=False,
+                     p=0.0, drop=None):
+    P = torch.empty_like(S)
+    Pd = torch.empty_like(S) if p > 0 else P
+    seed, off = drop if p > 0 else (0, 0)
+    call("mms2ut_attn_softmax_fwd_aug", S.data_ptr(), P.data_ptr(), Pd.data_ptr(), Z, Tq, Tk, ldS,
+         _p(key_mask), (key_mask.stride(0) if key_mask is not None else 0), int(extra_key), float(p), seed, off,
+         q_aug.data_ptr(), q_aug.stride(0), float(scale), int(n_img), u_aug.data_ptr(), u_aug.stride(0), int(npad),
+         _s())
+    return P, Pd
+
+
+def attn_softmax_bwd_aug(P, dPd, Z, Tq, Tk, ldS, du_aug, scale, n_img, dq_aug, npad, p=0.0, drop=None):
+    seed, off = drop if p > 0 else (0, 0)
+    call("mms2ut_attn_softmax_bwd_aug", P.data_ptr(), dPd.data_ptr(), dPd.data_ptr(), Z, Tq, Tk, ldS, float(p),
+         seed, off, du_aug.data_ptr(), du_aug.stride(0), float(scale), int(n_img), dq_aug.data_ptr(),
+         dq_aug.stride(0), int(npad), _s())
+    return dPd
+
 FLASH_HD = (64, 96, 128)
 
 
diff --git a/multimodal-s2ut_amd/model.py b/multimodal-s2ut_amd/model.py
--- a/multimodal-s2ut_amd/model.py
+++ b/multimodal-s2ut_amd/model.py
@@ -968,19 +968,37 @@
             Wo, bo = self.P(pre + ".proj.weight"), self.P(pre + ".proj.bias")
         c["pre"] = pre
         q = K.linear(textd, Wq, bq)
-        kv = K.linear(imgd, Wkv, bkv)
-        if extra:
-            bkv_rows = self.params.span(pre + ".bias_k", pre + ".bias_v").view(1, 2 * d)
-            K.copy2d(bkv_rows.expand(B, 2 * d), kv.view(B, Tk * 2 * d)[:, Ti * 2 * d:], B, 2 * d)
-        c["q"], c["kv"] = q, kv
+        c["q"] = q
         key_mask = img_mask
         c["key_mask"] = key_mask
         pat = self._p("SA_attention_dropout")
         c["drop_attn"] = self._drop(pat, B * Te * Tk)
         O = torch.empty(B * Te, d, dtype=F16, device=text.device)
-        c["P"], c["Pd"], c["ldS"] = attn_fwd(q, kv, kv[:, d:], d, 2 * d, 2 * d, B, 1, Te, Tk, d,
-                                             d ** -0.5, O, d, key_mask=key_mask, extra_key=extra,
-                                             p=pat, drop=c["drop_attn"])
+        c["qs"] = self._fusion_call(Di).route(B, Te, Ti)
+        if c["qs"]:
+            R, Dia, ldS, scale = B * Te, K.round_up(Di + 2, 64), K.round_up(Tk, 8), d ** -0.5
+            waug = K.fusion_pack_kv(Wkv, bkv, self.params.span(pre + ".bias_k", pre + ".bias_v") if extra else None, Dia)
+            qk = torch.empty(R, Dia, dtype=F16, device=text.device)
+            K.gemm(q, waug, qk, R, Dia, d, b_kc=False, lda=d, ldb=Dia, ldc=Dia)
+            S = torch.empty(R * ldS, dtype=F16, device=text.device)
+            K.gemm(qk, imgd, S, Te, Tk, Di, lda=Dia, ldb=Di, ldc=ldS, batch=B, sA=(Te * Dia, 0), sB=(Tk * Di, 0),
+                   sC=(Te * ldS, 0), alpha=scale)
+            U = torch.empty(R, Dia, dtype=F16, device=text.device)
+            c["P"], c["Pd"] = K.attn_softmax_aug(S, B, Te, Tk, ldS, qk[:, Di:], scale, Ti, U[:, Di:], Dia - Di,
+                                                 key_mask=key_mask, extra_key=extra, p=pat, drop=c["drop_attn"])
+            K.gemm(c["Pd"], imgd, U, Te, Di, Tk, a_kc=True, b_kc=False, lda=ldS, ldb=Di, ldc=Dia, batch=B,
+                   sA=(Te * ldS, 0), sB=(Tk * Di, 0), sC=(Te * Dia, 0))
+            K.gemm(U, waug[d:], O, R, d, Dia, lda=Dia, ldb=Dia, ldc=d)
+            c["ldS"], c["waug"], c["qk"], c["U"] = ldS, waug, qk, U
+        else:
+            kv = K.linear(imgd, Wkv, bkv)
+            if extra:
+                bkv_rows = self.params.span(pre + ".bias_k", pre + ".bias_v").view(1, 2 * d)
+                K.copy2d(bkv_rows.expand(B, 2 * d), kv.view(B, Tk * 2 * d)[:, Ti * 2 * d:], B, 2 * d)
+            c["kv"] = kv
+            c["P"], c["Pd"], c["ldS"] = attn_fwd(q, kv, kv[:, d:], d, 2 * d, 2 * d, B, 1, Te, Tk, d,
+                                                 d ** -0.5, O, d, key_mask=key_mask, extra_key=extra,
+                                                 p=pat, drop=c["drop_attn"])
         c["O"], c["pat"], c["pimg"], c["ptxt"] = O, pat, pimg, ptxt
         if cfg["use_selective_gate"]:
             merge = torch.empty(B * Te, 2 * d, dtype=F16, device=text.device)
@@ -1031,29 +1049,58 @@
         K.linear_wgrad(dOp, c["O"], gWo,
                        db=gbo)
         dO = K.linear_dgrad(dOp, Wo)
-        q, kv = c["q"], c["kv"]
+        q = c["q"]
         dq = torch.empty_like(q)
-        dkv = torch.empty_like(kv)
-        attn_bwd(dO, d, q, kv, kv[:, d:], d, 2 * d, 2 * d, c["P"], c["Pd"], c["ldS"], B, 1, Te, Tk, d,
-                 d ** -0.5, dq, dkv, dkv[:, d:], d, 2 * d, 2 * d, p=c["pat"], drop=c["drop_attn"])
-        if extra:
-            rows = dkv.view(B, Tk * 2 * d)[:, Ti * 2 * d:]
-            K.bias_grad(rows, self.params.span(pre + ".bias_k", pre + ".bias_v", grad=True), side=False)
-            rows.zero_()
-        K.linear_wgrad(dkv, c["imgd"], gWkv,
-                       db=gbkv)
+        need_dx = bool(cfg["image_pre_norm"] or want_dimg)
+        dimgd = None
+        if c["qs"]:
+            R, Dia, ldS, scale = B * Te, c["waug"].shape[1], c["ldS"], d ** -0.5
+            waug, qk, U, imgd, P_, Pd = c["waug"], c["qk"], c["U"], c["imgd"], c["P"], c["Pd"]
+            dU = torch.empty(R, Dia, dtype=F16, device=dres.device)
+            K.gemm(dO, waug[d:], dU, R, Dia, d, b_kc=False, lda=d, ldb=Dia, ldc=Dia)
+            dwa = torch.empty(2 * d, Dia, dtype=F16, device=dres.device)
+            K.linear_wgrad(dO, U, dwa[d:])
+            dPd = torch.empty_like(P_)
+            K.gemm(dU, imgd, dPd, Te, Tk, Di, lda=Dia, ldb=Di, ldc=ldS, batch=B, sA=(Te * Dia, 0), sB=(Tk * Di, 0),
+                   sC=(Te * ldS, 0))
+            dqk = torch.empty(R, Dia, dtype=F16, device=dres.device)
+            K.attn_softmax_bwd_aug(P_, dPd, B, Te, Tk, ldS, dU[:, Di:], scale, Ti, dqk[:, Di:], Dia - Di,
+                                   p=c["pat"], drop=c["drop_attn"])
+            K.gemm(dPd, imgd, dqk, Te, Di, Tk, a_kc=True, b_kc=False, lda=ldS, ldb=Di, ldc=Dia, batch=B,
+                   sA=(Te * ldS, 0), sB=(Tk * Di, 0), sC=(Te * Dia, 0), alpha=scale)
+            K.linear_wgrad(q, dqk, dwa[:d])
+            K.fusion_unpack_kv(dwa, gWkv, gbkv,
+                               self.params.span(pre + ".bias_k", pre + ".bias_v", grad=True) if extra else None)
+            K.gemm(dqk, waug[:d], dq, R, d, Dia, lda=Dia, ldb=Dia, ldc=d)
+            if need_dx:
+                dimgd = torch.empty(B * Tk, Di, dtype=F16, device=dres.device)
+                K.gemm(dPd, qk, dimgd, Tk, Di, Te, a_kc=False, b_kc=False, lda=ldS, ldb=Dia, ldc=Di, batch=B,
+                       sA=(Te * ldS, 0), sB=(Te * Dia, 0), sC=(Tk * Di, 0), alpha=scale)
+                K.gemm(Pd, dU, dimgd, Tk, Di, Te, a_kc=False, b_kc=False, lda=ldS, ldb=Dia, ldc=Di, batch=B,
+                       sA=(Te * ldS, 0), sB=(Te * Dia, 0), sC=(Tk * Di, 0), epi=K.EPI_F16_ACC)
+        else:
+            kv = c["kv"]
+            dkv = torch.empty_like(kv)
+            attn_bwd(dO, d, q, kv, kv[:, d:], d, 2 * d, 2 * d, c["P"], c["Pd"], c["ldS"], B, 1, Te, Tk, d,
+                     d ** -0.5, dq, dkv, dkv[:, d:], d, 2 * d, 2 * d, p=c["pat"], drop=c["drop_attn"])
+            if extra:
+                rows = dkv.view(B, Tk * 2 * d)[:, Ti * 2 * d:]
+                K.bias_grad(rows, self.params.span(pre + ".bias_k", pre + ".bias_v", grad=True), side=False)
+                rows.zero_()
+            K.linear_wgrad(dkv, c["imgd"], gWkv,
+                           db=gbkv)
+            if need_dx:
+                dimgd = K.linear_dgrad(dkv, Wkv)
         dimg_in = None
         if c["ln_fused"]:
-            dimgd = K.linear_dgrad(dkv, Wkv)
             dimg_in = K.layernorm_bwd(dimgd, c["img_in"], self.P("encoder.image_pre_norm_module.weight"), c["im"],
                                       c["ir"], self.params.span("encoder.image_pre_norm_module.weight",
                                                                 "encoder.image_pre_norm_module.bias", grad=True),
                                       want_dx=want_dimg, dy_grp=Ti if extra else 0, dy_grp_out=Tk if extra else 0,
                                       dy_p=c["pimg"], dy_drop=c["drop_img"])
-        elif cfg["image_pre_norm"] or want_dimg:
-            dimgd = K.linear_dgrad(dkv, Wkv)
+        elif need_dx:
             if extra:
-                dimg = torch.empty(B * Ti, Di, dtype=F16, device=dkv.device)
+                dimg = torch.empty(B * Ti, Di, dtype=F16, device=dimgd.device)
                 K.copy2d(dimgd.view(B, Tk * Di), dimg.view(B, Ti * Di), B, Ti * Di)
             else:
                 dimg = dimgd
```

New measurement: 2.011 million audio-frames/s, median of 6. 2.3% higher.
